# albertfgu/diffwave-sashimi

Measured on AMD Instinct MI355X. Metric: audio samples/sec (generate.py-style reverse-diffusion sampling, T=200), higher is better.
Workload: dtype f32-equivalent (3-term bf16 split, 6 products, fp32 accumulate); 1 GPU; wnet_h256_d36_T200; backbone=wavenet, batch_per_gpu=16, L=16000, T=200, parallelism=independent clips per GPU, no collective, sampler=hipGraph replay, on-device Philox noise

## Files before the change

### diffwave-sashimi_amd/_lib.py

```python
import ctypes
import os

HERE = os.path.dirname(os.path.abspath(__file__))
LIB_PATH = os.environ.get("DWS_LIB") or os.path.join(HERE, "libdws.so")

DWS_OK, DWS_ERR_INVALID, DWS_ERR_UNSUPPORTED, DWS_ERR_HIP, DWS_ERR_STATE = 0, -1, -2, -3, -4
DWS_KIND_WAVENET, DWS_KIND_SASHIMI = 1, 2
DWS_MAX_POOL = 8
DWS_SAMPLER_DDPM, DWS_SAMPLER_DDIM, DWS_SAMPLER_DPMPP2M = 0, 1, 2
DWS_START_AS_GIVEN, DWS_START_QSAMPLE = 0, 1

c_f32p = ctypes.c_void_p


class ModelDesc(ctypes.Structure):
    _fields_ = [
        ("kind", ctypes.c_int32),
        ("in_channels", ctypes.c_int32), ("out_channels", ctypes.c_int32),
        ("diffusion_step_embed_dim_in", ctypes.c_int32),
        ("diffusion_step_embed_dim_mid", ctypes.c_int32),
        ("diffusion_step_embed_dim_out", ctypes.c_int32),
        ("unconditional", ctypes.c_int32),
        ("mel_upsample", ctypes.c_int32 * 2),
        ("mel_bands", ctypes.c_int32),
        ("res_channels", ctypes.c_int32), ("skip_channels", ctypes.c_int32),
        ("num_res_layers", ctypes.c_int32), ("dilation_cycle", ctypes.c_int32),
        ("d_model", ctypes.c_int32), ("n_layers", ctypes.c_int32), ("n_pool", ctypes.c_int32),
        ("pool", ctypes.c_int32 * DWS_MAX_POOL), ("expand", ctypes.c_int32), ("ff", ctypes.c_int32),
        ("unet", ctypes.c_int32), ("L", ctypes.c_int32),
    ]


class SamplerEdit(ctypes.Structure):
    _fields_ = [
        ("edit_coef", ctypes.POINTER(ctypes.c_float)),
        ("known", c_f32p), ("mask", ctypes.c_void_p), ("known_noise", c_f32p), ("start_noise", c_f32p),
        ("start_step", ctypes.c_int32), ("start_mode", ctypes.c_int32),
    ]


_SIGS = {
    "dws_last_error": (ctypes.c_char_p, []),
    "dws_abi_version": (ctypes.c_int, []),
    "dws_arch": (ctypes.c_char_p, []),
    "dws_cauchy_sym_fwd": (ctypes.c_int, [c_f32p] * 4 + [ctypes.c_int64] * 3 + [ctypes.c_void_p]),
    "dws_cauchy_sym_bwd": (ctypes.c_int, [c_f32p] * 6 + [ctypes.c_int64] * 3 + [ctypes.c_void_p]),
    "dws_cauchy_fwd": (ctypes.c_int, [c_f32p] * 4 + [ctypes.c_int64] * 3 + [ctypes.c_void_p]),
    "dws_cauchy_bwd": (ctypes.c_int, [c_f32p] * 6 + [ctypes.c_int64] * 3 + [ctypes.c_void_p]),
    "dws_model_create": (ctypes.c_int, [ctypes.POINTER(ModelDesc), ctypes.POINTER(ctypes.c_void_p)]),
    "dws_model_destroy": (ctypes.c_int, [ctypes.c_void_p]),
    "dws_model_num_params": (ctypes.c_int, [ctypes.c_void_p]),
    "dws_model_param_info": (ctypes.c_int, [ctypes.c_void_p, ctypes.c_int, ctypes.POINTER(ctypes.c_char_p),
                                            ctypes.POINTER(ctypes.c_int64), ctypes.POINTER(ctypes.c_int),
                                            ctypes.POINTER(ctypes.c_int)]),
    "dws_model_set_param": (ctypes.c_int, [ctypes.c_void_p, ctypes.c_char_p, ctypes.c_void_p,
                                           ctypes.POINTER(ctypes.c_int64), ctypes.c_int, ctypes.c_int,
                                           ctypes.c_void_p]),
    "dws_model_update_params": (ctypes.c_int, [ctypes.c_void_p, ctypes.c_int32, ctypes.POINTER(ctypes.c_char_p),
                                               ctypes.POINTER(ctypes.c_void_p), ctypes.c_void_p]),
    "dws_model_set_option": (ctypes.c_int, [ctypes.c_void_p, ctypes.c_char_p, ctypes.c_char_p]),
    "dws_model_commit": (ctypes.c_int, [ctypes.c_void_p, ctypes.c_void_p]),
    "dws_model_prepare": (ctypes.c_int, [ctypes.c_void_p, ctypes.c_int64, ctypes.c_int64]),
    "dws_model_set_condition": (ctypes.c_int, [ctypes.c_void_p, c_f32p, ctypes.c_int64, ctypes.c_int64,
                                               ctypes.c_void_p]),
    "dws_model_forward": (ctypes.c_int, [ctypes.c_void_p, c_f32p, c_f32p, c_f32p, ctypes.c_void_p]),
    "dws_model_forward_train": (ctypes.c_int, [ctypes.c_void_p, c_f32p, c_f32p, c_f32p, ctypes.c_void_p]),
    "dws_model_backward": (ctypes.c_int, [ctypes.c_void_p, c_f32p, ctypes.c_void_p]),
    "dws_model_backward_input": (ctypes.c_int, [ctypes.c_void_p, c_f32p, c_f32p, ctypes.c_int32, ctypes.c_void_p]),
    "dws_model_get_grad": (ctypes.c_int, [ctypes.c_void_p, ctypes.c_char_p, c_f32p, ctypes.c_int64, ctypes.c_void_p]),
    "dws_model_get_grads": (ctypes.c_int, [ctypes.c_void_p, ctypes.c_int32, ctypes.POINTER(ctypes.c_char_p),
                                           ctypes.POINTER(ctypes.c_void_p), ctypes.POINTER(ctypes.c_int64), ctypes.c_void_p]),
    "dws_model_set_grad_sinks": (ctypes.c_int, [ctypes.c_void_p, ctypes.c_int32, ctypes.POINTER(ctypes.c_char_p),
                                                ctypes.POINTER(ctypes.c_void_p), ctypes.POINTER(ctypes.c_int64),
                                                ctypes.POINTER(ctypes.c_int32), ctypes.c_int32]),
    "dws_model_grad_group_wait": (ctypes.c_int, [ctypes.c_void_p, ctypes.c_int32, ctypes.c_void_p]),
    "dws_model_grad_ready_seq": (ctypes.c_int, [ctypes.c_void_p, ctypes.c_int32, ctypes.POINTER(ctypes.c_char_p),
                                                ctypes.POINTER(ctypes.c_int32)]),
    "dws_model_read_tap": (ctypes.c_int, [ctypes.c_void_p, ctypes.c_char_p, c_f32p, ctypes.c_int64, ctypes.c_void_p]),
    "dws_sampler_run": (ctypes.c_int, [ctypes.c_void_p, c_f32p, ctypes.POINTER(ctypes.c_float),
                                       ctypes.POINTER(ctypes.c_float), ctypes.POINTER(ctypes.c_float),
                                       ctypes.c_int32, c_f32p, ctypes.c_uint64, ctypes.c_int32, ctypes.c_int32,
                                       ctypes.c_void_p]),
    "dws_sampler_steps": (ctypes.c_int, [ctypes.c_void_p, c_f32p, ctypes.POINTER(ctypes.c_float),
                                         ctypes.POINTER(ctypes.c_float), ctypes.POINTER(ctypes.c_float),
                                         ctypes.c_int32, ctypes.c_int32, ctypes.c_int32, ctypes.c_uint64,
                                         ctypes.c_int32, ctypes.c_void_p]),
    "dws_sampler_run_schedule": (ctypes.c_int, [ctypes.c_void_p, c_f32p, ctypes.c_int32, ctypes.c_int32,
                                                ctypes.POINTER(ctypes.c_float), ctypes.POINTER(ctypes.c_float), c_f32p,
                                                ctypes.c_uint64, ctypes.c_int32, ctypes.c_int32, ctypes.c_void_p]),
    "dws_sampler_run_edit": (ctypes.c_int, [ctypes.c_void_p, c_f32p, ctypes.c_int32, ctypes.c_int32,
                                            ctypes.POINTER(ctypes.c_float), ctypes.POINTER(ctypes.c_float), c_f32p,
                                            ctypes.c_uint64, ctypes.c_int32, ctypes.c_int32,
                                            ctypes.POINTER(SamplerEdit), ctypes.c_void_p]),
    "dws_sampler_run_program": (ctypes.c_int, [ctypes.c_void_p, c_f32p, ctypes.c_int32, ctypes.c_int32,
                                               ctypes.POINTER(ctypes.c_float), ctypes.POINTER(ctypes.c_float),
                                               ctypes.c_int32, ctypes.POINTER(ctypes.c_int32),
                                               ctypes.POINTER(ctypes.c_float), c_f32p, ctypes.c_uint64, ctypes.c_int32,
                                               ctypes.c_int32, ctypes.POINTER(SamplerEdit), ctypes.c_void_p]),
    "dws_philox_normal": (ctypes.c_int, [c_f32p, ctypes.c_int64, ctypes.c_uint64, ctypes.c_uint32, ctypes.c_void_p]),
    "dws_mel_spectrogram": (ctypes.c_int, [c_f32p, ctypes.c_int64, ctypes.c_int64, c_f32p, c_f32p, ctypes.c_int32,
                                           ctypes.c_int32, ctypes.c_int32, ctypes.c_float, c_f32p, ctypes.c_void_p]),
    "dws_gemm_bf16x6": (ctypes.c_int, [c_f32p] * 3 + [ctypes.c_int64] * 3 + [ctypes.c_void_p]),
    "dws_gemm_f16x3": (ctypes.c_int, [c_f32p] * 3 + [ctypes.c_int64] * 3 + [ctypes.c_float] * 2 + [ctypes.c_void_p]),
    "dws_profile_enable": (ctypes.c_int, [ctypes.c_char_p]),
    "dws_profile_query": (ctypes.c_int, [ctypes.POINTER(ctypes.c_int64), ctypes.POINTER(ctypes.c_double)]),
    "dws_profile_query_each": (ctypes.c_int, [ctypes.POINTER(ctypes.c_double), ctypes.c_int64, ctypes.POINTER(ctypes.c_int64)]),
    "dws_profile_disable": (ctypes.c_int, []),
}

EXPORTS = tuple(_SIGS)

_lib = None


def load():
    global _lib
    if _lib is not None:
        return _lib
    if not os.path.exists(LIB_PATH):
        raise RuntimeError(
            f"{LIB_PATH} not found: the HIP engine is not built (run `python -c 'import __graft_entry__ as g; "
            "g.build()'`).  There is no CPU fallback.")
    lib = ctypes.CDLL(LIB_PATH, mode=ctypes.RTLD_GLOBAL)
    for name, (res, args) in _SIGS.items():
        fn = getattr(lib, name)
        fn.restype, fn.argtypes = res, args
    _lib = lib
    return lib


def check(status):
    if status == DWS_OK:
        return
    msg = load().dws_last_error().decode("utf-8", "replace")
    if status == DWS_ERR_UNSUPPORTED:
        raise NotImplementedError(msg)
    raise RuntimeError(f"libdws error {status}: {msg}")


def ptr(t):
    return 0 if t is None else t.data_ptr()


def current_stream():
    import torch
    return torch.cuda.current_stream().cuda_stream
```

### diffwave-sashimi_amd/csrc/bf16_split.h

```cpp
#pragma once
#include <hip/hip_runtime.h>

namespace dws {

typedef __bf16 bx_bf16x8 __attribute__((ext_vector_type(8)));
typedef __bf16 bx_bf16x4 __attribute__((ext_vector_type(4)));
typedef float bx_f32x16 __attribute__((ext_vector_type(16)));

__device__ __forceinline__ void split3(float x, __bf16& p0, __bf16& p1, __bf16& p2) {
    p0 = (__bf16)x;
    const float r1 = x - (float)p0;
    p1 = (__bf16)r1;
    const float r2 = r1 - (float)p1;
    p2 = (__bf16)r2;
}

__device__ __forceinline__ void split3x4(const float (&x)[4], bx_bf16x4& p0, bx_bf16x4& p1, bx_bf16x4& p2) {
#pragma unroll
    for (int e = 0; e < 4; ++e) {
        __bf16 a, b, c;
        split3(x[e], a, b, c);
        p0[e] = a; p1[e] = b; p2[e] = c;
    }
}

__device__ constexpr int BX6_IA[6] = {2, 1, 0, 1, 0, 0};
__device__ constexpr int BX6_IB[6] = {0, 1, 2, 0, 1, 0};

__device__ __forceinline__ void mfma6(bx_f32x16& acc, const bx_bf16x8 (&a)[3], const bx_bf16x8 (&b)[3]) {
#pragma unroll
    for (int t = 0; t < 6; ++t) acc = __builtin_amdgcn_mfma_f32_32x32x16_bf16(a[BX6_IA[t]], b[BX6_IB[t]], acc, 0, 0, 0);
}

__device__ __forceinline__ void frag_rank2(float v0, float v1, bool lower_half, bx_bf16x8 (&out)[3]) {
    __bf16 a0, a1, a2, b0, b1, b2;
    split3(lower_half ? v0 : 0.f, a0, a1, a2);
    split3(lower_half ? v1 : 0.f, b0, b1, b2);
    const __bf16 z = (__bf16)0.f;
    out[0] = bx_bf16x8{a0, b0, z, z, z, z, z, z};
    out[1] = bx_bf16x8{a1, b1, z, z, z, z, z, z};
    out[2] = bx_bf16x8{a2, b2, z, z, z, z, z, z};
}

struct SplitBf16x3 {
    typedef bx_bf16x8 v8;
    typedef bx_bf16x4 v4;
    static constexpr int NT = 3, NP = 6;
    static constexpr bool SCALED = false;
    static constexpr float SX = 1.f, SG = 1.f;
    __device__ static constexpr int ia(int t) { return BX6_IA[t]; }
    __device__ static constexpr int ib(int t) { return BX6_IB[t]; }
    __device__ static __forceinline__ bx_f32x16 mfma(const v8& a, const v8& b, const bx_f32x16& c) {
        return __builtin_amdgcn_mfma_f32_32x32x16_bf16(a, b, c, 0, 0, 0);
    }
    __device__ static __forceinline__ void split4(const float (&x)[4], v4 (&p)[3]) { split3x4(x, p[0], p[1], p[2]); }
    __device__ static __forceinline__ void split1(float x, v8 (&out)[3], int i) {
        __bf16 a, b, c;
        split3(x, a, b, c);
        out[0][i] = a; out[1][i] = b; out[2][i] = c;
    }
    __device__ static __forceinline__ void rank2(float v0, float v1, bool lower_half, v8 (&out)[3]) { frag_rank2(v0, v1, lower_half, out); }
    __device__ static __forceinline__ void bits(float x, unsigned short (&b)[3]) {
        __bf16 p0, p1, p2;
        split3(x, p0, p1, p2);
        b[0] = __builtin_bit_cast(unsigned short, p0); b[1] = __builtin_bit_cast(unsigned short, p1); b[2] = __builtin_bit_cast(unsigned short, p2);
    }
    __device__ static __forceinline__ v8 bvals(float v0, float v1) {
        const __bf16 z = (__bf16)0.f;
        return v8{(__bf16)v0, (__bf16)v1, z, z, z, z, z, z};
    }
};

typedef _Float16 hx_f16x8 __attribute__((ext_vector_type(8)));
typedef _Float16 hx_f16x4 __attribute__((ext_vector_type(4)));
struct SplitF16x2 {
    typedef hx_f16x8 v8;
    typedef hx_f16x4 v4;
    static constexpr int NT = 2, NP = 3;
    static constexpr bool SCALED = true;
#ifndef F16X3_SX
#define F16X3_SX 16.f
#endif
    static constexpr float SX = F16X3_SX, SG = 4096.f;
    __device__ static constexpr int ia(int t) { return t == 0 ? 1 : 0; }
    __device__ static constexpr int ib(int t) { return t == 1 ? 1 : 0; }
    __device__ static __forceinline__ bx_f32x16 mfma(const v8& a, const v8& b, const bx_f32x16& c) {
        return __builtin_amdgcn_mfma_f32_32x32x16_f16(a, b, c, 0, 0, 0);
    }
    __device__ static __forceinline__ void split4(const float (&x)[4], v4 (&p)[2]) {
#pragma unroll
        for (int e = 0; e < 4; ++e) {
            const _Float16 h = (_Float16)x[e];
            p[0][e] = h;
            p[1][e] = (_Float16)(x[e] - (float)h);
        }
    }
    __device__ static __forceinline__ void split1(float x, v8 (&out)[2], int i) {
        const _Float16 h = (_Float16)x;
        out[0][i] = h;
        out[1][i] = (_Float16)(x - (float)h);
    }
    __device__ static __forceinline__ void bits(float x, unsigned short (&b)[2]) {
        const _Float16 h = (_Float16)x, l = (_Float16)(x - (float)h);
        b[0] = __builtin_bit_cast(unsigned short, h); b[1] = __builtin_bit_cast(unsigned short, l);
    }
    __device__ static __forceinline__ void rank2(float v0, float v1, bool lower_half, v8 (&out)[2]) {
        const _Float16 z = (_Float16)0.f;
        out[0] = v8{z, z, z, z, z, z, z, z};
        out[1] = out[0];
        split1(lower_half ? v0 : 0.f, out, 0);
        split1(lower_half ? v1 : 0.f, out, 1);
    }
    __device__ static __forceinline__ v8 bvals(float v0, float v1) {
        const _Float16 z = (_Float16)0.f;
        return v8{(_Float16)v0, (_Float16)v1, z, z, z, z, z, z};
    }
};

}
```

### diffwave-sashimi_amd/csrc/wavenet.h

```cpp
#pragma once
#include "dws_common.h"

namespace dws {

constexpr int WN_LAYER_KC = 32;
constexpr int WN_BX3_KC = 16;

struct WnLayerArgs {
    const float* x_in;
    float* x_out;
    float* skip;
    const float* part_t;
    int part_t_bstride;
    const float* A1;
    const float* A2;
    const float* Abt;
    int abt_bstride;
    const int* step_idx;
    int abt_tstride, part_t_tstride;
    const float* Wd;
    const float* Wr;
    const float* Ws;
    const float* bias1;
    const float* bias2;
    const float* melc;
    int mel_bstride;
    float* gate_ws;
    float* hsave;
    int B, L, dilation, first_layer, last_layer;
    const float* wscale;
    unsigned long long* trace;
};

struct WnFinalArgs {
    const float* skip;
    const float* Af;
    const float* Wf;
    const float* bf;
    const float* Wz;
    const float* bz;
    float* out;
    float* tap;
    float scale;
    int B, L, Cout;
    int af_scaled;
};

int launch_fold_weight_norm(const float* v, const float* g, float* out, int O, int inner, hipStream_t s);
int launch_permute_dconv(const float* w, float* out, int C, int KC, hipStream_t s);
int launch_pack_a_frag(const float* w, float* out, int M, int K, hipStream_t s);
int launch_pack_a_frag_t(const float* w, float* out, int O, int K, hipStream_t s);
int launch_step_embed(const float* steps, const float* freq, float* emb, int B, int half, hipStream_t s);
int launch_iota_f32(float* out, int n, hipStream_t s);
int launch_linear_rows(const float* in, const float* W, const float* bias, float* out, int B, int K, int O,
                       int act, hipStream_t s, float* pre_out = nullptr);
int launch_init_conv_bwd_data(const float* g, const float* y, const float* W, float* daudio, int B, int Cin, int C, int L,
                              hipStream_t s);
int launch_init_conv(const float* audio, const float* W, const float* bias, float* x, int B, int Cin, int C, int L,
                     hipStream_t s);
int launch_wn_bias_tap(const float* Wd_all, const float* part_t, float* Abt, int NL, int B, int C, hipStream_t s);
bool wn_layer_mfma_supported(int C, int S);
int launch_wn_layer_mfma(int C, int S, const WnLayerArgs& a, hipStream_t s);
int launch_wn_layer_generic(int C, int S, const WnLayerArgs& a, hipStream_t s);
bool wn_final_mfma_supported(int S);
bool wn_layer_wino_supported(int C, int S);
int launch_wino_dconv(const float* w, float* out, int C, hipStream_t s);
int launch_wn_wino_bias(const float* Wd_all, const float* part_t, float* Abt, int NL, int B, int C, hipStream_t s);
int launch_wn_layer_wino(int C, int S, const WnLayerArgs& a, hipStream_t s);
bool wn_layer_bf16x3_supported(int C, int S);
int launch_wn_layer_bf16x3(int C, int S, const WnLayerArgs& a, hipStream_t s);
int launch_pack_a_bf16x3(const float* w, void* out, int M, int K, hipStream_t s);
int launch_wn_bias_tap_bf16(const float* Wd_all, const float* part_t, const float* bias1_all, void* Abt, int NL, int B, int C,
                            hipStream_t s);
enum { WN_SPLIT_BF16X6 = 0, WN_SPLIT_F16X3 = 1 };
inline int wn_split_terms(int split) { return split == WN_SPLIT_F16X3 ? 2 : 3; }
bool wn_layer_bx6_supported(int C, int S);
int launch_wn_layer_bx6(int C, int S, const WnLayerArgs& a, int split, hipStream_t s);
int launch_weight_scale(const float* w, size_t n, const float* bias, int nb, const float* bias_b, int nb_b, float* out, hipStream_t s);
int launch_pack_a1_bx6(const float* w, void* out, int C, int split, const float* scale, hipStream_t s);
int launch_pack_a_bx6(const float* w, void* out, int M, int K, int split, const float* scale, hipStream_t s);
int launch_gemm_bx6(const float* A, const float* B, float* C, int M, int N, int K, int split, float sa, float sb, hipStream_t s);
int launch_wn_final(int S, const WnFinalArgs& a, hipStream_t s);

}
```

### diffwave-sashimi_amd/csrc/wavenet_bx6.hip

```cpp
#include <cstdlib>
#include <type_traits>

#include "bf16_split.h"
#include "wavenet.h"
#include "wn_trace.h"

namespace dws {

#ifndef BX6_PF3
#define BX6_PF3 1
#endif
#ifndef BX6_PF2
#define BX6_PF2 2
#endif
#define BX6_PF(NT) ((NT) == 2 ? BX6_PF2 : BX6_PF3)
#ifndef BX6_T_PER_MFMA
#define BX6_T_PER_MFMA 7
#endif

typedef float bx6_f32x4 __attribute__((ext_vector_type(4)));

#ifdef BX6_ABL_NO_NT
#define BX6_NT 0
#else
#define BX6_NT 2
#endif
__device__ __forceinline__ bx6_f32x4 bx6_load_f4(__amdgpu_buffer_rsrc_t r, int voff, int soff) {
    return __builtin_bit_cast(bx6_f32x4, __builtin_amdgcn_raw_buffer_load_b128(r, voff, soff, BX6_NT));
}
__device__ __forceinline__ void bx6_store_f4(bx6_f32x4 v, __amdgpu_buffer_rsrc_t r, int voff, int soff) {
    typedef unsigned int u4 __attribute__((ext_vector_type(4)));
    __builtin_amdgcn_raw_buffer_store_b128(__builtin_bit_cast(u4, v), r, voff, soff, BX6_NT);
}

__device__ __forceinline__ float bx6_gate(float t, float s) {
    const float tc = __builtin_amdgcn_fmed3f(t, -30.f, 30.f);
    const float e2 = __builtin_amdgcn_exp2f(tc * 2.8853900817779268f);
    const float en = __builtin_amdgcn_exp2f(s * -1.4426950408889634f);
    return (e2 - 1.f) * __builtin_amdgcn_rcpf((e2 + 1.f) * (1.f + en));
}

template <typename P>
__global__ void pack_a1_bx6_kernel(const float* __restrict__ w, unsigned short* __restrict__ out, int C, const float* __restrict__ scale) {
    const size_t i = (size_t)blockIdx.x * blockDim.x + threadIdx.x;
    if (i >= (size_t)2 * C * C * 4) return;
    const int e = (int)(i & 7), lane = (int)((i >> 3) & 63), j = (int)((i >> 9) & 3);
    const size_t r = i >> 11;
    const int nkb = C / 16;
    const int kb = (int)(r % nkb), mt = (int)(r / nkb);
    const int o = mt * 32 + (lane & 31), c = kb * 16 + 8 * (lane >> 5) + e;
    const float* wr = w + ((size_t)o * C + c) * 3;
    const float w0 = wr[0], w1 = wr[1], w2 = wr[2];
    float g;
    if (j == 0) g = w0;
    else if (j == 1) g = 0.5f * ((w0 + w2) + w1);
    else if (j == 2) g = 0.5f * ((w0 + w2) - w1);
    else g = w2;
    if (P::SCALED) g *= *scale;
    unsigned short b[P::NT];
    P::bits(g, b);
    const size_t base = ((r * 4 + j) * P::NT) * 512 + (size_t)lane * 8 + e;
#pragma unroll
    for (int t = 0; t < P::NT; ++t) out[base + t * 512] = b[t];
}

template <typename P>
__global__ void pack_a_bx6_kernel(const float* __restrict__ w, unsigned short* __restrict__ out, int M, int K, const float* __restrict__ scale) {
    const size_t i = (size_t)blockIdx.x * blockDim.x + threadIdx.x;
    if (i >= (size_t)M * K) return;
    const int e = (int)(i & 7), lane = (int)((i >> 3) & 63);
    const size_t r = i >> 9;
    const int nkb = K / 16;
    const int kb = (int)(r % nkb), mt = (int)(r / nkb);
    float v = w[(size_t)(mt * 32 + (lane & 31)) * K + kb * 16 + 8 * (lane >> 5) + e];
    if (P::SCALED) v *= *scale;
    unsigned short b[P::NT];
    P::bits(v, b);
    const size_t base = (r * P::NT) * 512 + (size_t)lane * 8 + e;
#pragma unroll
    for (int t = 0; t < P::NT; ++t) out[base + t * 512] = b[t];
}

__global__ __launch_bounds__(1024) void weight_scale_kernel(const float* __restrict__ w, size_t n, const float* __restrict__ bias, int nb,
                                                            const float* __restrict__ bias_b, int nb_b, float* __restrict__ out) {
    __shared__ float red[16];
    float m = 0.f;
    for (size_t i = threadIdx.x; i < n; i += 1024) m = fmaxf(m, fabsf(w[i]));
    if (bias)
        for (int i = threadIdx.x; i < nb; i += 1024) m = fmaxf(m, fabsf(bias[i]) * (1.f / 1024.f));
    if (bias_b)
        for (int i = threadIdx.x; i < nb_b; i += 1024) m = fmaxf(m, fabsf(bias_b[i]) * (1.f / 1024.f));
#pragma unroll
    for (int o = 32; o > 0; o >>= 1) m = fmaxf(m, __shfl_xor(m, o));
    if ((threadIdx.x & 63) == 0) red[threadIdx.x >> 6] = m;
    __syncthreads();
    if (threadIdx.x == 0) {
        for (int i = 1; i < 16; ++i) m = fmaxf(m, red[i]);
        int ex = 0;
        if (m > 0.f && m < 3.0e38f) {
            frexpf(m, &ex);
            if (ex > 100) ex = 100;
            if (ex < -100) ex = -100;
        }
        *out = ldexpf(1.f, 1 - ex);
    }
}

int launch_weight_scale(const float* w, size_t n, const float* bias, int nb, const float* bias_b, int nb_b, float* out, hipStream_t s) {
    hipLaunchKernelGGL(weight_scale_kernel, dim3(1), dim3(1024), 0, s, w, n, bias, nb, bias_b, nb_b, out);
    return DWS_OK;
}

int launch_pack_a1_bx6(const float* w, void* out, int C, int split, const float* scale, hipStream_t s) {
    const size_t n = (size_t)2 * C * C * 4;
    if (split == WN_SPLIT_F16X3) {
        DWS_CHECK(scale != nullptr, DWS_ERR_INVALID, "pack_a1: the fp16 split needs the matrix scale");
        hipLaunchKernelGGL(pack_a1_bx6_kernel<SplitF16x2>, dim3(ceil_div(n, 256)), dim3(256), 0, s, w, (unsigned short*)out, C, scale);
    } else {
        hipLaunchKernelGGL(pack_a1_bx6_kernel<SplitBf16x3>, dim3(ceil_div(n, 256)), dim3(256), 0, s, w, (unsigned short*)out, C, scale);
    }
    return DWS_OK;
}

int launch_pack_a_bx6(const float* w, void* out, int M, int K, int split, const float* scale, hipStream_t s) {
    DWS_CHECK(M % 32 == 0 && K % 16 == 0, DWS_ERR_UNSUPPORTED, "pack_a_bx6: M=%d K=%d", M, K);
    const size_t n = (size_t)M * K;
    if (split == WN_SPLIT_F16X3) {
        DWS_CHECK(scale != nullptr, DWS_ERR_INVALID, "pack_a: the fp16 split needs the matrix scale");
        hipLaunchKernelGGL(pack_a_bx6_kernel<SplitF16x2>, dim3(ceil_div(n, 256)), dim3(256), 0, s, w, (unsigned short*)out, M, K, scale);
    } else {
        hipLaunchKernelGGL(pack_a_bx6_kernel<SplitBf16x3>, dim3(ceil_div(n, 256)), dim3(256), 0, s, w, (unsigned short*)out, M, K, scale);
    }
    return DWS_OK;
}

template <int C, int S, int NT>
struct Bx6Tile {
    static constexpr int WAVES = C / 32;
    static constexpr int NTH = WAVES * 64;
    static constexpr int NP = 32;
    static constexpr int KC = (C >= 256) ? 32 : 16;
    static constexpr int NCB = C / KC;
    static constexpr int NKB = C / 16;
    static constexpr int MS = S / C;
    static constexpr int RAW_FLOATS = KC * 4 * NP;
    static constexpr int BOP_BYTES = (KC / 8) * 4 * NT * NP * 16;
    static constexpr int STAGE_FLOATS = 2 * RAW_FLOATS + 2 * BOP_BYTES / 4;
    static constexpr int GATE_BYTES = (C / 8) * NT * 64 * 16;
    static constexpr int MAIN_FLOATS = STAGE_FLOATS > GATE_BYTES / 4 ? STAGE_FLOATS : GATE_BYTES / 4;
    static constexpr int TR_FLOATS = 32 * 64;
    static constexpr int LDS_FLOATS = MAIN_FLOATS + WAVES * TR_FLOATS;
    static constexpr int TITEMS = (KC / 4) * NP * 2;
    static_assert(C % 32 == 0 && S % C == 0 && C % KC == 0 && KC % 16 == 0 && KC % (2 * WAVES) == 0 &&
                  (TITEMS % NTH == 0) && LDS_FLOATS * 4 <= 163840, "channel counts");
};

template <typename P, int C, int S, bool EXTRA>
__global__ __launch_bounds__(C * 2, (C >= 128 ? 2 : 1)) void wn_layer_bx6_kernel(WnLayerArgs a, int log2d) {
    using T = Bx6Tile<C, S, P::NT>;
    using v8 = typename P::v8;
    using v4 = typename P::v4;
    constexpr int NT = P::NT, NPR = P::NP, NA = 2 * P::NT;
    constexpr int KC = T::KC, MS = T::MS, WAVES = T::WAVES, NCB = T::NCB, NTH = T::NTH, NKB = T::NKB;
    __shared__ __attribute__((aligned(16))) float lds[T::LDS_FLOATS];
    float* const Xraw = lds;
    char* const Bop = reinterpret_cast<char*>(lds + 2 * T::RAW_FLOATS);
    char* const gt = reinterpret_cast<char*>(lds);

    const int tid = threadIdx.x;
    const int lane = tid & 63;
    const int wave = __builtin_amdgcn_readfirstlane(tid >> 6);
    const int l31 = lane & 31, lhi = lane >> 5;
    const int L = a.L, dil = 1 << log2d;
    float* const trw = lds + T::MAIN_FLOATS + wave * T::TR_FLOATS;

    const int nblk = (L + 2 * dil - 1) >> (log2d + 1);
    const int ntl = ((nblk << log2d) + 31) >> 5;
    const int tile = xcd_remap(blockIdx.x, gridDim.x);
    const int b = __builtin_amdgcn_readfirstlane(tile / ntl);
    const int tic = tile % ntl;
#ifdef WN_TILE_ORDER_LINEAR
    const int q0 = __builtin_amdgcn_readfirstlane(tic * 32);
#else
    const int q0 = __builtin_amdgcn_readfirstlane(log2d >= 6 ? ((tic % nblk) << log2d) + (tic / nblk) * 32 : tic * 32);
#endif
    const int q = q0 + l31;
    const int p = ((q >> log2d) << (log2d + 1)) + (q & (dil - 1));

    const float* __restrict__ xb = a.x_in + (size_t)b * C * L;
    unsigned long long* __restrict__ trc = a.trace ? a.trace + ((size_t)blockIdx.x * WAVES + wave) * 32 : nullptr;
    auto stamp = [&](int i) {
        if (trc) {
            const unsigned long long t = __builtin_amdgcn_s_memtime();
            if (lane == 0) trc[i] = t;
        }
    };
    stamp(0);

    const int mt1[2] = {wave, C / 32 + wave};
    int mt2[1 + MS];
    mt2[0] = wave;
#pragma unroll
    for (int m = 0; m < MS; ++m) mt2[1 + m] = C / 32 + wave * MS + m;
    float av1[2][4], ab1[2], av2[1 + MS];
    {
        const float* Abt = a.Abt + (size_t)b * a.abt_bstride + step_row_off(a.step_idx, a.abt_tstride);
#pragma unroll
        for (int m = 0; m < 2; ++m) {
            const int row = mt1[m] * 32 + l31;
#pragma unroll
            for (int j = 0; j < 4; ++j) av1[m][j] = Abt[j * 2 * C + row];
            ab1[m] = a.bias1[row];
        }
#pragma unroll
        for (int m = 0; m < 1 + MS; ++m) av2[m] = a.bias2[mt2[m] * 32 + l31];
    }
    const float ws1 = P::SCALED ? a.wscale[0] : 1.f, ws2 = P::SCALED ? a.wscale[1] : 1.f;
    const float inv1 = 1.f / (ws1 * P::SX), inv2 = 1.f / (ws2 * P::SG);

    const bool al16 = (L % 4 == 0) && ((((size_t)a.x_in | (size_t)a.x_out | (size_t)a.skip) & 15) == 0);
    const bool contig = al16 && log2d <= 4;
    const bool x4 = contig || (al16 && log2d >= 2);
    constexpr int RPW = KC / WAVES;
    __amdgpu_buffer_rsrc_t rXall = __builtin_amdgcn_make_buffer_rsrc((void*)xb, 0, C * L * 4, 0x00020000);
    const int pbase = (q0 >> log2d) << (log2d + 1);
    const int ob = contig ? 32 + (p - pbase) - dil : l31;
    const int os = contig ? dil : 32;
    const int x0l = p - pbase, x1l = x0l + dil;
    const int gcol0 = contig ? x0l : l31, gcol1 = contig ? x1l : 32 + l31;
    int voffA, voffB;
    if (contig) {
        const int pp = pbase - 32 + 4 * (lane & 31);
        voffA = ((unsigned)pp < (unsigned)L) ? (lhi * L + pp) * 4 : 0x7ffffff0;
        voffB = 0;
    } else if (x4) {
        const int s4 = (lane >> 3) & 3, qq = q0 + 4 * (lane & 7);
        const int pp = ((qq >> log2d) << (log2d + 1)) + (qq & (dil - 1)) + (s4 - 1) * dil;
        voffA = ((unsigned)pp < (unsigned)L) ? (lhi * L + pp) * 4 : 0x7ffffff0;
        voffB = 0;
    } else {
        voffA = (p + (lhi - 1) * dil) * 4;
        voffB = (p + (lhi + 1) * dil) * 4;
    }
#ifdef BX6_ABL_NO_ROT
    const int rot = 0;
#else
    const int rot = __builtin_amdgcn_readfirstlane((int)((unsigned)tic % NCB));
#endif
    auto chunk_of = [&](int cb) { const int c = cb + rot; return c >= NCB ? c - NCB : c; };
    constexpr int NPIECE = RPW / 2;
    auto stage_piece = [&](int cbi, int i) {
        float* xs = Xraw + (cbi & 1) * T::RAW_FLOATS;
        const int cb = chunk_of(cbi);
        {
            const int cc = 2 * (wave + WAVES * i);
            if (x4) {
                __builtin_amdgcn_raw_ptr_buffer_load_lds(rXall, xs + cc * 128, 16, voffA, (cb * KC + cc) * L * 4, 0, BX6_NT);
            } else {
#pragma unroll
                for (int h = 0; h < 2; ++h) {
                    __amdgpu_buffer_rsrc_t r = __builtin_amdgcn_make_buffer_rsrc((void*)(xb + (size_t)(cb * KC + cc + h) * L), 0, L * 4, 0x00020000);
                    __builtin_amdgcn_raw_ptr_buffer_load_lds(r, xs + (cc + h) * 128, 4, voffA, 0, 0, 0);
                    __builtin_amdgcn_raw_ptr_buffer_load_lds(r, xs + (cc + h) * 128 + 64, 4, voffB, 0, 0, 0);
                }
            }
        }
    };
    auto stage_dma = [&](int cbi) {
#pragma unroll
        for (int i = 0; i < NPIECE; ++i) stage_piece(cbi, i);
    };

    auto transform = [&](int c1) {
        const float* xs = Xraw + (c1 & 1) * T::RAW_FLOATS;
        char* bo = Bop + (c1 & 1) * T::BOP_BYTES;
#pragma unroll
        for (int k = 0; k < T::TITEMS / NTH; ++k) {
            const int i = tid + NTH * k;
            const int gi = __builtin_amdgcn_readfirstlane(i >> 6);
            const int g4 = (gi * 2 + lhi) % (KC / 4);
            const int jp = __builtin_amdgcn_readfirstlane((gi * 2) / (KC / 4));
            float ta[4], tb[4];
#pragma unroll
            for (int e = 0; e < 4; ++e) {
                const float* xr = xs + (g4 * 4 + e) * 128 + ob;
                const float d1 = xr[os], d2 = xr[2 * os];
                if (jp == 0) {
                    const float d0 = xr[0];
                    ta[e] = d0 - d2; tb[e] = d1 + d2;
                } else {
                    const float d3 = xr[3 * os];
                    ta[e] = d2 - d1; tb[e] = d1 - d3;
                }
            }
            if (P::SCALED) {
#pragma unroll
                for (int e = 0; e < 4; ++e) { ta[e] *= P::SX; tb[e] *= P::SX; }
            }
            v4 pa[NT], pb[NT];
            P::split4(ta, pa);
            P::split4(tb, pb);
            char* dst = bo + ((((g4 >> 1) * 4 + 2 * jp) * NT) * 32 + l31) * 16 + (g4 & 1) * 8;
#pragma unroll
            for (int t = 0; t < NT; ++t) {
                *reinterpret_cast<v4*>(dst + t * 512) = pa[t];
                *reinterpret_cast<v4*>(dst + (NT + t) * 512) = pb[t];
            }
        }
        if (al16) {
            const int ch0 = chunk_of(c1) * KC;
            if (ch0 / 32 == wave) {
                const int r0 = ch0 % 32;
#pragma unroll
                for (int i = 0; i < KC / 4; ++i) {
                    const int rr = (lane >> 4) + 4 * i;
                    const bx6_f32x4 v = *reinterpret_cast<const bx6_f32x4*>(xs + rr * 128 + 32 + 4 * (lane & 15));
                    *reinterpret_cast<bx6_f32x4*>(trw + (r0 + rr) * 64 + 4 * (lane & 15)) = v;
                }
            }
        }
    };

    bx_f32x16 acc[2][4];
    __amdgpu_buffer_rsrc_t rA1 = __builtin_amdgcn_make_buffer_rsrc((void*)a.A1, 0, 2 * C * 4 * C * 2 * NT, 0x00020000);
    const int lane16 = lane * 16;
    auto load_a1 = [&](v8 (&dst)[2][NT], int kb, int j) {
#pragma unroll
        for (int m = 0; m < 2; ++m)
#pragma unroll
            for (int t = 0; t < NT; ++t)
#ifdef BX6_ABL_A_HOT
                dst[m][t] = __builtin_bit_cast(v8, __builtin_amdgcn_raw_buffer_load_b128(rA1, lane16, ((mt1[m] * NKB * 4) * NT + t) * 1024 + 0 * (kb + j), 0));
#else
                dst[m][t] = __builtin_bit_cast(v8, __builtin_amdgcn_raw_buffer_load_b128(rA1, lane16, (((mt1[m] * NKB + kb) * 4 + j) * NT + t) * 1024, 0));
#endif
    };

    stage_dma(0);
    if (NCB > 1) stage_dma(1);
    constexpr int PF = BX6_PF(NT);
    v8 a_ring[4][2][NT];
#pragma unroll
    for (int s0 = 0; s0 < PF; ++s0) load_a1(a_ring[s0], chunk_of(0) * (KC / 16) + (s0 >> 2), s0 & 3);
    constexpr int NAF = PF * NA;
    if (NCB > 1) {
        if (x4) __builtin_amdgcn_s_waitcnt(0x0F70 | ((RPW / 2 + NAF) & 15) | (((RPW / 2 + NAF) >> 4) << 14));
        else __builtin_amdgcn_s_waitcnt(0x0F70 | ((2 * RPW + NAF) & 15) | (((2 * RPW + NAF) >> 4) << 14));
    } else {
        __builtin_amdgcn_s_waitcnt(0x0F70 | NAF);
    }
    __syncthreads();
    stamp(1);
    {
        const float v0 = ((unsigned)(p - dil) < (unsigned)L) ? 1.f : 0.f;
        const float v1 = ((unsigned)p < (unsigned)L) ? 1.f : 0.f;
        const float v2 = ((unsigned)(p + dil) < (unsigned)L) ? 1.f : 0.f;
        const float v3 = ((unsigned)(p + 2 * dil) < (unsigned)L) ? 1.f : 0.f;
        const float bi[4] = {v0 - v2, v1 + v2, v2 - v1, v1 - v3};
        bx_f32x16 zero;
#pragma unroll
        for (int r = 0; r < 16; ++r) zero[r] = 0.f;
#pragma unroll
        for (int j = 0; j < 4; ++j) {
            const v8 bf = P::bvals(lhi ? 0.f : bi[j] * P::SX, (lhi || j != 1) ? 0.f : P::SX);
#pragma unroll
            for (int m = 0; m < 2; ++m) {
                v8 af[NT];
                P::rank2(av1[m][j] * ws1, j == 1 ? ab1[m] * ws1 : 0.f, lhi == 0, af);
                acc[m][j] = zero;
#pragma unroll
                for (int t = NT - 1; t >= 0; --t) acc[m][j] = P::mfma(af[t], bf, acc[m][j]);
            }
        }
    }
    transform(0);
    __builtin_amdgcn_s_waitcnt(0x0F70 | NAF);
    __syncthreads();

    constexpr int SPC = (KC / 16) * 4;
    auto do_step = [&](int cb, auto ST, auto WITH_T) {
        constexpr int st = decltype(ST)::value;
        constexpr bool with_t = decltype(WITH_T)::value;
        constexpr int it = st >> 2, j = st & 3;
        constexpr int sn = (st + PF) % SPC, itn = sn >> 2, jn = sn & 3;
        const int cbn = cb + (st + PF) / SPC;
        const char* tb = Bop + (cb & 1) * T::BOP_BYTES + lhi * (4 * NT * 512) + l31 * 16;
#if !defined(BX6_ABL_NO_STAGE) && defined(BX6_STAGE_SPREAD)
        if (cb + 2 < NCB) {
            constexpr int NS = (SPC - PF) < 1 ? 1 : (SPC - PF);
#pragma unroll
            for (int i = 0; i < NPIECE; ++i)
                if (i * NS / NPIECE == st) stage_piece(cb + 2, i);
        }
#endif
        if (cbn < NCB) load_a1(a_ring[(st + PF) & 3], chunk_of(cbn) * (KC / 16) + itn, jn);
        __builtin_amdgcn_sched_barrier(0);
        v8 bq[NT];
#pragma unroll
        for (int t = 0; t < NT; ++t) bq[t] = *reinterpret_cast<const v8*>(tb + ((2 * it * 4 + j) * NT + t) * 512);
#ifndef BX6_ABL_NO_TRANSFORM
        if (with_t) transform(cb + 1);
#endif
#pragma unroll
        for (int t = 0; t < NPR; ++t)
#pragma unroll
            for (int m = 0; m < 2; ++m)
                acc[m][j] = P::mfma(a_ring[st & 3][m][P::ia(t)], bq[P::ib(t)], acc[m][j]);
#ifndef BX6_ABL_NO_INTERLEAVE
        if (with_t) {
#pragma unroll
            for (int i = 0; i < 2 * NPR; ++i) {
                __builtin_amdgcn_sched_group_barrier(0x008, 1, 0);
                __builtin_amdgcn_sched_group_barrier(0x302, BX6_T_PER_MFMA * 6 / NPR, 0);
            }
        }
#endif
    };
    auto do_steps_from1 = [&](int cb) {
        if constexpr (SPC == 4) {
            do_step(cb, std::integral_constant<int, 1>{}, std::false_type{});
            do_step(cb, std::integral_constant<int, 2>{}, std::false_type{});
            do_step(cb, std::integral_constant<int, 3>{}, std::false_type{});
        } else {
            do_step(cb, std::integral_constant<int, 1>{}, std::false_type{});
            do_step(cb, std::integral_constant<int, 2>{}, std::false_type{});
            do_step(cb, std::integral_constant<int, 3>{}, std::false_type{});
            do_step(cb, std::integral_constant<int, 4>{}, std::false_type{});
            do_step(cb, std::integral_constant<int, 5>{}, std::false_type{});
            do_step(cb, std::integral_constant<int, 6>{}, std::false_type{});
            do_step(cb, std::integral_constant<int, 7>{}, std::false_type{});
        }
    };
    static_assert((SPC == 4 || SPC == 8) && PF >= 1 && PF <= 3, "steps per chunk, prefetch distance");
    for (int cb = 0; cb < NCB; ++cb) {
#if !defined(BX6_ABL_NO_STAGE) && !defined(BX6_STAGE_SPREAD)
        if (cb + 2 < NCB) stage_dma(cb + 2);
#endif
        if (cb + 1 < NCB) do_step(cb, std::integral_constant<int, 0>{}, std::true_type{});
        else do_step(cb, std::integral_constant<int, 0>{}, std::false_type{});
        do_steps_from1(cb);
        stamp(8 + 2 * cb);
#ifndef BX6_ABL_NO_DMA_WAIT
        __builtin_amdgcn_s_waitcnt(0x0F70 | NAF);
#endif
#ifndef BX6_ABL_NO_BARRIER
        __syncthreads();
#endif
        stamp(9 + 2 * cb);
    }
    stamp(2);

    const int L4 = L * 4;
    const bool first = a.first_layer, last = a.last_layer;
    __amdgpu_buffer_rsrc_t rXo = __builtin_amdgcn_make_buffer_rsrc((void*)(a.x_out + (size_t)b * C * L), 0, C * L * 4, 0x00020000);
    __amdgpu_buffer_rsrc_t rSk = __builtin_amdgcn_make_buffer_rsrc((void*)(a.skip + (size_t)b * S * L), 0, S * L * 4, 0x00020000);
    const int p0 = ((q0 >> log2d) << (log2d + 1)) + (q0 & (dil - 1));
    int voff4;
    {
        const int n4 = (lane & 15) >> 3;
        const int pos4 = (contig ? pbase + 32 * n4 : p0 + n4 * dil) + 4 * (lane & 7);
        voff4 = (pos4 < L) ? ((lane >> 4) * L + pos4) * 4 : 0x7ffffff0;
    }
    constexpr bool PRELOAD = MS == 1;
    const int voff4s = first ? 0x7ffffff0 : voff4;
    auto load_pre = [&](int m, bx6_f32x4 (&dst)[8]) {
#pragma unroll
        for (int i = 0; i < 8; ++i) {
            if (m == 0) dst[i] = *reinterpret_cast<const bx6_f32x4*>(trw + ((lane >> 4) + 4 * i) * 64 + 4 * (lane & 15));
            else dst[i] = bx6_load_f4(rSk, voff4s, ((wave * MS + (m - 1)) * 32 + 4 * i) * L4);
        }
    };
    bx6_f32x4 pre[PRELOAD ? 1 + MS : 1][8];
    if (PRELOAD && al16) {
#pragma unroll
        for (int m = 1; m < 1 + MS; ++m) load_pre(m, pre[PRELOAD ? m : 0]);
    }

    const float* melb = (EXTRA && a.melc) ? a.melc + (size_t)(a.mel_bstride ? b : 0) * 2 * C * L : nullptr;
#pragma unroll
    for (int qd = 0; qd < 4; ++qd) {
        float g0[4], g1[4];
#pragma unroll
        for (int e = 0; e < 4; ++e) {
            const int r = qd * 4 + e;
            const int ch = wave * 32 + e + 8 * qd + 4 * lhi;
#pragma unroll
            for (int n = 0; n < 2; ++n) {
                const int pos = p + n * dil;
                float ht, hs;
                if (n == 0) {
                    ht = (acc[0][0][r] + acc[0][1][r]) + acc[0][2][r];
                    hs = (acc[1][0][r] + acc[1][1][r]) + acc[1][2][r];
                } else {
                    ht = (acc[0][1][r] - acc[0][2][r]) - acc[0][3][r];
                    hs = (acc[1][1][r] - acc[1][2][r]) - acc[1][3][r];
                }
                if (P::SCALED) { ht *= inv1; hs *= inv1; }
                if (EXTRA && melb && pos < L) {
                    ht += melb[(size_t)ch * L + pos];
                    hs += melb[(size_t)(C + ch) * L + pos];
                }
                if (EXTRA && a.hsave && pos < L) {
                    float* __restrict__ hb = a.hsave + (size_t)b * 2 * C * L;
                    hb[(size_t)ch * L + pos] = ht;
                    hb[(size_t)(C + ch) * L + pos] = hs;
                }
                const float g = bx6_gate(ht, hs) * P::SG;
                if (n == 0) g0[e] = g; else g1[e] = g;
            }
        }
        v4 s0[NT], s1[NT];
        P::split4(g0, s0);
        P::split4(g1, s1);
        char* dst = gt + ((wave * 4 + qd) * NT * 64) * 16 + lhi * 8;
#pragma unroll
        for (int t = 0; t < NT; ++t) {
            *reinterpret_cast<v4*>(dst + (t * 64 + gcol0) * 16) = s0[t];
            *reinterpret_cast<v4*>(dst + (t * 64 + gcol1) * 16) = s1[t];
        }
    }
    stamp(3);

    __amdgpu_buffer_rsrc_t rA2 = __builtin_amdgcn_make_buffer_rsrc((void*)a.A2, 0, (C + S) * C * 2 * NT, 0x00020000);
    v8 c_cur[1 + MS][NT], c_nxt[1 + MS][NT];
    auto load_a2 = [&](v8 (&dst)[1 + MS][NT], int kb) {
#pragma unroll
        for (int m = 0; m < 1 + MS; ++m)
#pragma unroll
            for (int t = 0; t < NT; ++t)
                dst[m][t] = __builtin_bit_cast(v8, __builtin_amdgcn_raw_buffer_load_b128(rA2, lane16, ((mt2[m] * NKB + kb) * NT + t) * 1024, 0));
    };
    const int rot2 = rot * (KC / 16);
    auto kblock_of = [&](int kb) { const int k = kb + rot2; return k >= NKB ? k - NKB : k; };
    load_a2(c_cur, kblock_of(0));
    bx_f32x16 acc2[1 + MS][2];
    {
        const v8 bf = P::bvals(lhi ? 0.f : P::SG, 0.f);
        bx_f32x16 zero;
#pragma unroll
        for (int r = 0; r < 16; ++r) zero[r] = 0.f;
#pragma unroll
        for (int m = 0; m < 1 + MS; ++m) {
            v8 af[NT];
            P::rank2(av2[m] * ws2, 0.f, lhi == 0, af);
#pragma unroll
            for (int n = 0; n < 2; ++n) {
                acc2[m][n] = zero;
#pragma unroll
                for (int t = NT - 1; t >= 0; --t) acc2[m][n] = P::mfma(af[t], bf, acc2[m][n]);
            }
        }
    }
    __syncthreads();
    stamp(4);
    const char* gb = gt + lhi * (NT * 64 * 16) + l31 * 16;
#pragma unroll 2
    for (int kb = 0; kb < NKB; ++kb) {
        const int kbn = (kb + 1 < NKB) ? kb + 1 : kb;
        load_a2(c_nxt, kblock_of(kbn));
        __builtin_amdgcn_sched_barrier(0);
        const char* gk = gb + kblock_of(kb) * (2 * NT * 64 * 16);
        v8 bq[2][NT];
#pragma unroll
        for (int n = 0; n < 2; ++n)
#pragma unroll
            for (int t = 0; t < NT; ++t) bq[n][t] = *reinterpret_cast<const v8*>(gk + (t * 64 + n * 32) * 16);
#pragma unroll
        for (int t = 0; t < NPR; ++t)
#pragma unroll
            for (int m = 0; m < 1 + MS; ++m)
#pragma unroll
                for (int n = 0; n < 2; ++n)
                    acc2[m][n] = P::mfma(c_cur[m][P::ia(t)], bq[n][P::ib(t)], acc2[m][n]);
#pragma unroll
        for (int m = 0; m < 1 + MS; ++m)
#pragma unroll
            for (int t = 0; t < NT; ++t) c_cur[m][t] = c_nxt[m][t];
    }
    stamp(5);

    const float rs = 0.70710678118654752440f;
    if (al16) {
#pragma unroll
        for (int m = 0; m < 1 + MS; ++m) {
            if (m == 0 && last) continue;
            if (!PRELOAD || m == 0) load_pre(m, pre[0]);
            asm volatile("s_waitcnt lgkmcnt(0)" ::: "memory");
#pragma unroll
            for (int n = 0; n < 2; ++n)
#pragma unroll
                for (int r = 0; r < 16; ++r) trw[((r & 3) + 8 * (r >> 2) + 4 * lhi) * 64 + n * 32 + l31] = P::SCALED ? acc2[m][n][r] * inv2 : acc2[m][n][r];
            asm volatile("s_waitcnt lgkmcnt(0)" ::: "memory");
            const int row0 = (m == 0) ? wave * 32 : (wave * MS + (m - 1)) * 32;
#pragma unroll
            for (int i = 0; i < 8; ++i) {
                const bx6_f32x4 v = *reinterpret_cast<const bx6_f32x4*>(trw + ((lane >> 4) + 4 * i) * 64 + 4 * (lane & 15));
                bx6_f32x4 o = pre[PRELOAD ? m : 0][i] + v;
                if (m == 0) o = o * rs;
                bx6_store_f4(o, m == 0 ? rXo : rSk, voff4, (row0 + 4 * i) * L4);
                asm volatile("s_nop 1" ::: "memory");
            }
            asm volatile("" ::: "memory");
        }
    } else {
        int voffn[2];
#pragma unroll
        for (int n = 0; n < 2; ++n) {
            const int pos = contig ? pbase + 32 * n + l31 : p + n * dil;
            voffn[n] = (pos < L) ? (4 * lhi * L + pos) * 4 : 0x7ffffff0;
        }
#pragma unroll
        for (int n = 0; n < 2; ++n) {
            if (!last) {
                const int s0 = (wave * 32) * L4;
#pragma unroll
                for (int r = 0; r < 16; ++r) {
                    const int so = s0 + ((r & 3) + 8 * (r >> 2)) * L4;
                    const float x = __builtin_bit_cast(float, __builtin_amdgcn_raw_buffer_load_b32(rXall, voffn[n], so, 0));
                    const float v = (x + (P::SCALED ? acc2[0][n][r] * inv2 : acc2[0][n][r])) * rs;
                    __builtin_amdgcn_raw_buffer_store_b32(__builtin_bit_cast(unsigned, v), rXo, voffn[n], so, 0);
                }
            }
#pragma unroll
            for (int m = 0; m < MS; ++m) {
                const int s0 = ((wave * MS + m) * 32) * L4;
#pragma unroll
                for (int r = 0; r < 16; ++r) {
                    const int so = s0 + ((r & 3) + 8 * (r >> 2)) * L4;
                    const float old = first ? 0.f : __builtin_bit_cast(float, __builtin_amdgcn_raw_buffer_load_b32(rSk, voffn[n], so, 0));
                    const float v = old + (P::SCALED ? acc2[1 + m][n][r] * inv2 : acc2[1 + m][n][r]);
                    __builtin_amdgcn_raw_buffer_store_b32(__builtin_bit_cast(unsigned, v), rSk, voffn[n], so, 0);
                }
            }
        }
    }
    stamp(6);
    if (trc) {
        __builtin_amdgcn_s_waitcnt(0);
        stamp(7);
    }
}

template <typename P, int C, int S>
static int launch_bx6_t(const WnLayerArgs& a, int log2d, hipStream_t s) {
    ProfileScope ps(P::NT == 3 ? "wn_layer_bx6" : "wn_layer_f16x3", s);
    using T = Bx6Tile<C, S, P::NT>;
    const int dil = 1 << log2d;
    const int nblk = (a.L + 2 * dil - 1) / (2 * dil);
    const int ntl = (nblk * dil + 31) / 32;
    const int ntiles = a.B * ntl;
    static const bool trace = std::getenv("DWS_BX6_TRACE") != nullptr;
    if (trace && !a.melc && !a.hsave) {
        wino_trace_launch(ntiles, T::WAVES, a, s, [&](const WnLayerArgs& at) {
            hipLaunchKernelGGL((wn_layer_bx6_kernel<P, C, S, false>), dim3(ntiles), dim3(T::NTH), 0, s, at, log2d);
        }, P::NT == 3 ? "bx6" : "f16x3");
        return DWS_OK;
    }
    if (a.melc || a.hsave) hipLaunchKernelGGL((wn_layer_bx6_kernel<P, C, S, true>), dim3(ntiles), dim3(T::NTH), 0, s, a, log2d);
    else hipLaunchKernelGGL((wn_layer_bx6_kernel<P, C, S, false>), dim3(ntiles), dim3(T::NTH), 0, s, a, log2d);
    return DWS_OK;
}

bool wn_layer_bx6_supported(int C, int S) {
    return (C == 64 && S == 64) || (C == 128 && S == 128) || (C == 128 && S == 256) || (C == 256 && S == 256);
}

template <typename P>
static int launch_bx6_p(int C, int S, const WnLayerArgs& a, int log2d, hipStream_t s) {
    if (C == 64 && S == 64) return launch_bx6_t<P, 64, 64>(a, log2d, s);
    if (C == 128 && S == 128) return launch_bx6_t<P, 128, 128>(a, log2d, s);
    if (C == 128 && S == 256) return launch_bx6_t<P, 128, 256>(a, log2d, s);
    if (C == 256 && S == 256) return launch_bx6_t<P, 256, 256>(a, log2d, s);
    return set_error(DWS_ERR_UNSUPPORTED, "wn_layer_bx6: (C=%d,S=%d) not instantiated", C, S);
}

int launch_wn_layer_bx6(int C, int S, const WnLayerArgs& a, int split, hipStream_t s) {
    int log2d = 0;
    while ((1 << log2d) < a.dilation) ++log2d;
    DWS_CHECK((1 << log2d) == a.dilation, DWS_ERR_UNSUPPORTED, "wn_layer_bx6: dilation %d is not a power of two", a.dilation);
    DWS_CHECK((int64_t)a.L + 4 * (int64_t)a.dilation < ((int64_t)1 << 28), DWS_ERR_UNSUPPORTED, "wn_layer_bx6: L too large");
    DWS_CHECK((int64_t)(C > S ? C : S) * a.L * 4 < ((int64_t)1 << 31), DWS_ERR_UNSUPPORTED,
              "wn_layer_bx6: %d channels x L=%d exceed a 2 GiB tensor per clip", C > S ? C : S, a.L);
    if (split == WN_SPLIT_F16X3) {
        DWS_CHECK(a.hsave == nullptr, DWS_ERR_UNSUPPORTED, "wn_layer_f16x3: the training forward runs with precision=f32 or bf16x6");
        DWS_CHECK(a.wscale != nullptr, DWS_ERR_INVALID, "wn_layer_f16x3: no weight scales");
        return launch_bx6_p<SplitF16x2>(C, S, a, log2d, s);
    }
    return launch_bx6_p<SplitBf16x3>(C, S, a, log2d, s);
}

template <typename P>
__global__ __launch_bounds__(64) void gemm_bx6_kernel(const float* __restrict__ A, const float* __restrict__ B, float* __restrict__ Cm,
                                                      int M, int N, int K, float sa, float sb) {
    using v8 = typename P::v8;
    const int lane = threadIdx.x, l31 = lane & 31, lhi = lane >> 5;
    const int mt = blockIdx.y, nt = blockIdx.x;
    bx_f32x16 acc;
#pragma unroll
    for (int r = 0; r < 16; ++r) acc[r] = 0.f;
    for (int kb = 0; kb < K / 16; ++kb) {
        v8 af[P::NT], bf[P::NT];
#pragma unroll
        for (int e = 0; e < 8; ++e) {
            const int k = kb * 16 + 8 * lhi + e;
            P::split1(A[(size_t)(mt * 32 + l31) * K + k] * sa, af, e);
            P::split1(B[(size_t)k * N + nt * 32 + l31] * sb, bf, e);
        }
#pragma unroll
        for (int t = 0; t < P::NP; ++t) acc = P::mfma(af[P::ia(t)], bf[P::ib(t)], acc);
    }
    const float inv = 1.f / (sa * sb);
#pragma unroll
    for (int r = 0; r < 16; ++r)
        Cm[(size_t)(mt * 32 + (r & 3) + 8 * (r >> 2) + 4 * lhi) * N + nt * 32 + l31] = acc[r] * inv;
}

int launch_gemm_bx6(const float* A, const float* B, float* Cm, int M, int N, int K, int split, float sa, float sb, hipStream_t s) {
    DWS_CHECK(M > 0 && N > 0 && K > 0 && M % 32 == 0 && N % 32 == 0 && K % 16 == 0, DWS_ERR_UNSUPPORTED,
              "gemm_bf16x6 / gemm_f16x3: M=%d N=%d must be multiples of 32, K=%d of 16", M, N, K);
    if (split == WN_SPLIT_F16X3) {
        int ea = 0, eb = 0;
        DWS_CHECK(sa > 0.f && sb > 0.f && frexpf(sa, &ea) == 0.5f && frexpf(sb, &eb) == 0.5f, DWS_ERR_INVALID,
                  "gemm_f16x3: the operand scales must be powers of two (%g, %g)", (double)sa, (double)sb);
        hipLaunchKernelGGL(gemm_bx6_kernel<SplitF16x2>, dim3(N / 32, M / 32), dim3(64), 0, s, A, B, Cm, M, N, K, sa, sb);
    } else {
        hipLaunchKernelGGL(gemm_bx6_kernel<SplitBf16x3>, dim3(N / 32, M / 32), dim3(64), 0, s, A, B, Cm, M, N, K, 1.f, 1.f);
    }
    return DWS_OK;
}

}

extern "C" int dws_gemm_bf16x6(const float* A, const float* B, float* C, int64_t M, int64_t N, int64_t K, void* stream) {
    DWS_CHECK(A && B && C, DWS_ERR_INVALID, "dws_gemm_bf16x6: null argument");
    DWS_CHECK(M <= (1 << 20) && N <= (1 << 20) && K <= (1 << 20), DWS_ERR_UNSUPPORTED, "dws_gemm_bf16x6: dimension too large");
    return dws::launch_gemm_bx6(A, B, C, (int)M, (int)N, (int)K, dws::WN_SPLIT_BF16X6, 1.f, 1.f, (hipStream_t)stream);
}

extern "C" int dws_gemm_f16x3(const float* A, const float* B, float* C, int64_t M, int64_t N, int64_t K, float scale_a, float scale_b,
                              void* stream) {
    DWS_CHECK(A && B && C, DWS_ERR_INVALID, "dws_gemm_f16x3: null argument");
    DWS_CHECK(M <= (1 << 20) && N <= (1 << 20) && K <= (1 << 20), DWS_ERR_UNSUPPORTED, "dws_gemm_f16x3: dimension too large");
    return dws::launch_gemm_bx6(A, B, C, (int)M, (int)N, (int)K, dws::WN_SPLIT_F16X3, scale_a, scale_b, (hipStream_t)stream);
}
```

### diffwave-sashimi_amd/csrc/wavenet_model.hip

```cpp
#include <cmath>

#include "conditioner.h"
#include "model.h"
#include "wavenet.h"
#include "wavenet_backward.h"

namespace dws {

struct WaveNetModel : dws_model {
    int Cin, Cout, C, S, NL, cycle, Ein, Emid, Eout, MB;
    bool cond, mfma_layer, mfma_final;
    bool bf16x3 = false;
    bool bf16x6 = false;
    bool f16x3 = false;
    DevBuf wscale;
    bool wino_opt = true;
    bool wino_fits(int64_t nL) const {
        return (int64_t)std::max(C, S) * nL * 4 < ((int64_t)1 << 31) && nL + 4 * ((int64_t)1 << (cycle - 1)) < ((int64_t)1 << 28);
    }
    bool wino() const { return wino_opt && mfma_layer && !bf16x3 && !bf16x6 && !f16x3 && wn_layer_wino_supported(C, S) && (L == 0 || wino_fits(L)); }
    bool wino_rows() const { return wino() || bf16x6 || f16x3; }

    DevBuf Wi;
    std::vector<DevBuf> A1, Wrs, A2, bias2;
    DevBuf Wd_all;
    DevBuf Abt;
    DevBuf Wt_all, bt_all;
    DevBuf b1_all;
    DevBuf Wf, Af;
    DevBuf freq;
    CopyBatch stack_params, unstack_fc_t;
    bool freq_ready = false;
    DevBuf tmp_pack;
    std::vector<DevBuf> melW0, melW1, melWc;
    DevBuf melc;
    DevBuf mel_u0, mel_u1;
    int64_t melBm = 0;
    DevBuf mel_in;
    int mel_T = 0;
    CondTrainWs cws;
    DevBuf gW0f, gW1f, gWcf;
    DevBuf x0, x1, skip, gate, emb, h1, h2, part_t, scratch_out;
    std::vector<DevBuf> tx, tH;
    std::vector<DevBuf> ATd, ATg;
    std::vector<DevBuf> ATw;
    DevBuf ATf, wpart, bpart;
    bool mfma_bwd = false;
    uint64_t commit_version = 0, bwd_pack_version = ~0ull;
    DevBuf ty, ta1, ta2, dxa, dxb, dskip, dgb, dHb, dresb, dyb, dWfold, dpt, dh2, dh1, demb, dWt_all, dbt_all;
    bool trained_fwd = false;

    explicit WaveNetModel(const dws_model_desc& dd) {
        d = dd;
        Cin = d.in_channels; Cout = d.out_channels; C = d.res_channels; S = d.skip_channels;
        NL = d.num_res_layers; cycle = d.dilation_cycle;
        Ein = d.diffusion_step_embed_dim_in; Emid = d.diffusion_step_embed_dim_mid; Eout = d.diffusion_step_embed_dim_out;
        MB = d.mel_bands;
        cond = !d.unconditional;
        mfma_layer = wn_layer_mfma_supported(C, S);
        mfma_bwd = tapconv_mfma_supported(C, S, C, 1) && tapconv_mfma_supported(C, 2 * C, 0, 3) &&
                   tapconv_mfma_supported(S, S, 0, 1) && std::getenv("DWS_WAVENET_GENERIC_BWD") == nullptr;
        mfma_final = wn_final_mfma_supported(S);
        if (std::getenv("DWS_WN_DIRECT")) wino_opt = false;
        auto wn = [&](const std::string& p, std::vector<int64_t> vshape) {
            std::vector<int64_t> g(vshape.size(), 1);
            g[0] = vshape[0];
            add_param(p + ".bias", {vshape[0]});
            add_param(p + ".weight_g", g);
            add_param(p + ".weight_v", vshape);
        };
        wn("init_conv.0.conv", {C, Cin, 1});
        add_param("residual_layer.fc_t1.weight", {Emid, Ein});
        add_param("residual_layer.fc_t1.bias", {Emid});
        add_param("residual_layer.fc_t2.weight", {Eout, Emid});
        add_param("residual_layer.fc_t2.bias", {Eout});
        for (int n = 0; n < NL; ++n) {
            const std::string p = "residual_layer.residual_blocks." + std::to_string(n);
            add_param(p + ".fc_t.weight", {C, Eout});
            add_param(p + ".fc_t.bias", {C});
            wn(p + ".dilated_conv_layer.conv", {2 * C, C, 3});
            if (cond) {
                for (int i = 0; i < 2; ++i) {
                    const std::string u = p + ".upsample_conv2d." + std::to_string(i);
                    const int s = d.mel_upsample[i];
                    add_param(u + ".bias", {1});
                    add_param(u + ".weight_g", {1, 1, 1, 1});
                    add_param(u + ".weight_v", {1, 1, 3, 2 * s});
                }
                wn(p + ".mel_conv.conv", {2 * C, MB, 1});
            }
            wn(p + ".res_conv", {C, C, 1});
            wn(p + ".skip_conv", {S, C, 1});
        }
        wn("final_conv.0.conv", {S, S, 1});
        add_param("final_conv.2.conv.weight", {Cout, S, 1});
        add_param("final_conv.2.conv.bias", {Cout});
        A1.resize(NL); Wrs.resize(NL); A2.resize(NL); bias2.resize(NL);
        if (cond) { melW0.resize(NL); melW1.resize(NL); melWc.resize(NL); }
    }

    int set_option(const std::string& key, const std::string& value) override {
        if (key == "precision") {
            if (value == "f32") { bf16x3 = bf16x6 = f16x3 = false; dirty = true; trained_fwd = false; return DWS_OK; }
            if (value == "bf16x3") {
                DWS_CHECK(wn_layer_bf16x3_supported(C, S), DWS_ERR_UNSUPPORTED,
                          "precision=bf16x3 is not built for (res_channels=%d, skip_channels=%d)", C, S);
                bf16x3 = true; bf16x6 = f16x3 = false; dirty = true; trained_fwd = false;
                return DWS_OK;
            }
            if (value == "bf16x6") {
                DWS_CHECK(mfma_layer && wn_layer_bx6_supported(C, S), DWS_ERR_UNSUPPORTED,
                          "precision=bf16x6 is not built for (res_channels=%d, skip_channels=%d)", C, S);
                bf16x6 = true; bf16x3 = f16x3 = false; dirty = true; trained_fwd = false;
                return DWS_OK;
            }
            if (value == "f16x3") {
                DWS_CHECK(mfma_layer && wn_layer_bx6_supported(C, S), DWS_ERR_UNSUPPORTED,
                          "precision=f16x3 is not built for (res_channels=%d, skip_channels=%d)", C, S);
                f16x3 = true; bf16x3 = bf16x6 = false; dirty = true; trained_fwd = false;
                return DWS_OK;
            }
        }
        if (key == "conv_algo") {
            if (value == "winograd") { wino_opt = true; dirty = true; trained_fwd = false; return DWS_OK; }
            if (value == "direct") { wino_opt = false; dirty = true; trained_fwd = false; return DWS_OK; }
        }
        return dws_model::set_option(key, value);
    }

    float* Wd(int n) const { return Wd_all.f() + (size_t)n * 2 * C * C * 3; }

    int fold(const std::string& p, float* out, int O, int inner, hipStream_t s) {
        return launch_fold_weight_norm(P(p + ".weight_v"), P(p + ".weight_g"), out, O, inner, s);
    }

    int commit(hipStream_t s) override {
        DWS_TRY(Wi.ensure((size_t)C * Cin * 4));
        DWS_TRY(fold("init_conv.0.conv", Wi.f(), C, Cin, s));
        DWS_TRY(Wt_all.ensure((size_t)NL * C * Eout * 4));
        DWS_TRY(bt_all.ensure((size_t)NL * C * 4));
        DWS_TRY(b1_all.ensure((size_t)NL * 2 * C * 4));
        DWS_TRY(Wd_all.ensure((size_t)NL * 2 * C * C * 3 * 4));
        if (mfma_layer) DWS_TRY(tmp_pack.ensure((size_t)2 * C * 4 * C * 4));
        stack_params.begin();
        for (int n = 0; n < NL; ++n) {
            const std::string p = "residual_layer.residual_blocks." + std::to_string(n);
            stack_params.add(P(p + ".fc_t.weight"), Wt_all.f() + (size_t)n * C * Eout, (size_t)C * Eout);
            stack_params.add(P(p + ".fc_t.bias"), bt_all.f() + (size_t)n * C, (size_t)C);
            stack_params.add(P(p + ".dilated_conv_layer.conv.bias"), b1_all.f() + (size_t)n * 2 * C, (size_t)2 * C);
            DWS_TRY(fold(p + ".dilated_conv_layer.conv", Wd(n), 2 * C, C * 3, s));
            DWS_TRY(Wrs[n].ensure((size_t)(C + S) * C * 4));
            DWS_TRY(fold(p + ".res_conv", Wrs[n].f(), C, C, s));
            DWS_TRY(fold(p + ".skip_conv", Wrs[n].f() + (size_t)C * C, S, C, s));
            DWS_TRY(bias2[n].ensure((size_t)(C + S) * 4));
            stack_params.add(P(p + ".res_conv.bias"), bias2[n].f(), (size_t)C);
            stack_params.add(P(p + ".skip_conv.bias"), bias2[n].f() + C, (size_t)S);
            if (mfma_layer && (bf16x6 || f16x3)) {
                const int split = f16x3 ? WN_SPLIT_F16X3 : WN_SPLIT_BF16X6;
                const size_t tb = 2 * (size_t)wn_split_terms(split);
                float* sc = nullptr;
                if (f16x3) {
                    DWS_TRY(wscale.ensure((size_t)NL * 2 * 4));
                    sc = wscale.f() + 2 * n;
                    DWS_TRY(launch_weight_scale(Wd(n), (size_t)2 * C * C * 3, P(p + ".dilated_conv_layer.conv.bias"), 2 * C, nullptr, 0, sc, s));
                    DWS_TRY(launch_weight_scale(Wrs[n].f(), (size_t)(C + S) * C, P(p + ".res_conv.bias"), C, P(p + ".skip_conv.bias"), S,
                                                sc + 1, s));
                }
                DWS_TRY(A1[n].ensure((size_t)2 * C * 4 * C * tb));
                DWS_TRY(A2[n].ensure((size_t)(C + S) * C * tb));
                DWS_TRY(launch_pack_a1_bx6(Wd(n), A1[n].p, C, split, sc, s));
                DWS_TRY(launch_pack_a_bx6(Wrs[n].f(), A2[n].p, C + S, C, split, f16x3 ? sc + 1 : nullptr, s));
            } else if (mfma_layer) {
                DWS_TRY(A1[n].ensure((size_t)2 * C * 4 * C * 4));
                if (wino()) DWS_TRY(launch_wino_dconv(Wd(n), tmp_pack.f(), C, s));
                else DWS_TRY(launch_permute_dconv(Wd(n), tmp_pack.f(), C, bf16x3 ? WN_BX3_KC : WN_LAYER_KC, s));
                DWS_TRY(A2[n].ensure((size_t)(C + S) * C * 4));
                if (wino()) {
                    DWS_TRY(launch_pack_a_frag(tmp_pack.f(), A1[n].f(), 2 * C, 4 * C, s));
                    DWS_TRY(launch_pack_a_frag(Wrs[n].f(), A2[n].f(), C + S, C, s));
                } else if (bf16x3) {
                    DWS_TRY(launch_pack_a_bf16x3(tmp_pack.f(), A1[n].p, 2 * C, 3 * C, s));
                    DWS_TRY(launch_pack_a_bf16x3(Wrs[n].f(), A2[n].p, C + S, C, s));
                } else {
                    DWS_TRY(launch_pack_a_frag(tmp_pack.f(), A1[n].f(), 2 * C, 3 * C, s));
                    DWS_TRY(launch_pack_a_frag(Wrs[n].f(), A2[n].f(), C + S, C, s));
                }
            }
            if (cond) {
                for (int i = 0; i < 2; ++i) {
                    const int sc = d.mel_upsample[i];
                    DevBuf& w = (i == 0) ? melW0[n] : melW1[n];
                    DWS_TRY(w.ensure((size_t)3 * 2 * sc * 4));
                    DWS_TRY(fold(p + ".upsample_conv2d." + std::to_string(i), w.f(), 1, 3 * 2 * sc, s));
                }
                DWS_TRY(melWc[n].ensure((size_t)2 * C * MB * 4));
                DWS_TRY(fold(p + ".mel_conv.conv", melWc[n].f(), 2 * C, MB, s));
            }
        }
        DWS_TRY(Wf.ensure((size_t)S * S * 4));
        DWS_TRY(fold("final_conv.0.conv", Wf.f(), S, S, s));
        if (mfma_final) {
            DWS_TRY(Af.ensure((size_t)S * S * 4));
            DWS_TRY(tmp_pack.ensure((size_t)std::max(2 * C * 4 * C, S * S) * 4));
            DWS_TRY(launch_scale(Wf.f(), tmp_pack.f(), (float)std::sqrt(1.0 / NL), (size_t)S * S, s));
            DWS_TRY(launch_pack_a_frag(tmp_pack.f(), Af.f(), S, S, s));
        }
        DWS_TRY(stack_params.run(s));
        if (!freq_ready) {
            const int half = Ein / 2;
            std::vector<float> f(half);
            const float e = (float)(-(std::log(10000.0) / (half - 1)));
            for (int i = 0; i < half; ++i) f[i] = (float)std::exp((double)((float)i * e));
            DWS_TRY(freq.ensure((size_t)half * 4));
            DWS_HIP(hipMemcpyAsync(freq.p, f.data(), (size_t)half * 4, hipMemcpyHostToDevice, s));
            DWS_HIP(hipStreamSynchronize(s));
            freq_ready = true;
        }
        if (Abt.p) DWS_HIP(hipMemsetAsync(Abt.p, 0, Abt.bytes, s));
        dirty = false;
        ++commit_version;
        melBm = 0;
        return DWS_OK;
    }

    int pack_bwd(hipStream_t s) {
        const float r2 = 0.70710678118654752440f;
        ATd.resize(NL); ATg.resize(NL); ATw.resize(NL);
        DWS_TRY(tmp_pack.ensure((size_t)std::max(std::max(8 * C * C, (S + C) * C), S * S) * 4));
        for (int n = 0; n < NL; ++n) {
            if (wino_opt && tapwino_mfma_supported(C, 2 * C, 1 << (n % cycle))) {
                DWS_TRY(ATw[n].ensure((size_t)8 * C * C * 4));
                DWS_TRY(launch_tapwino_pack_transposed(Wd(n), tmp_pack.f(), 2 * C, C, s));
                DWS_TRY(launch_pack_a_frag(tmp_pack.f(), ATw[n].f(), C, 8 * C, s));
            } else {
                ATw[n].release();
                DWS_TRY(ATd[n].ensure((size_t)6 * C * C * 4));
                DWS_TRY(launch_tapconv_pack_transposed(Wd(n), tmp_pack.f(), 2 * C, C, 3, 6 * C, 0, 1.f, s));
                DWS_TRY(launch_pack_a_frag(tmp_pack.f(), ATd[n].f(), C, 6 * C, s));
            }
            DWS_TRY(ATg[n].ensure((size_t)(S + C) * C * 4));
            DWS_TRY(launch_tapconv_pack_transposed(Wrs[n].f() + (size_t)C * C, tmp_pack.f(), S, C, 1, S + C, 0, 1.f, s));
            DWS_TRY(launch_tapconv_pack_transposed(Wrs[n].f(), tmp_pack.f(), C, C, 1, S + C, S, r2, s));
            DWS_TRY(launch_pack_a_frag(tmp_pack.f(), ATg[n].f(), C, S + C, s));
        }
        DWS_TRY(ATf.ensure((size_t)S * S * 4));
        DWS_TRY(launch_tapconv_pack_transposed(Wf.f(), tmp_pack.f(), S, S, 1, S, 0, (float)std::sqrt(1.0 / NL), s));
        DWS_TRY(launch_pack_a_frag(tmp_pack.f(), ATf.f(), S, S, s));
        bwd_pack_version = commit_version;
        return DWS_OK;
    }

    int wgrad(const float* dY, const float* X, const float* addc, int addc_bs, float* dW, int O, int Cc, int T, int dil,
              float scale, hipStream_t s, float* db = nullptr, float bscale = 1.f) {
        if (!mfma_bwd) {
            if (db) DWS_TRY(launch_rowsum(dY, db, (int)B, O, (int)L, bscale, 0, s));
            return launch_wgrad(dY, X, addc, addc_bs, dW, (int)B, O, Cc, (int)L, T, dil, scale, s);
        }
        WgradArgs w{};
        w.dY = dY; w.X = X; w.addc = addc; w.addc_bstride = addc_bs;
        w.B = (int)B; w.O = O; w.C = Cc; w.L = (int)L; w.dil = dil;
        w.split = (bf16x6 && O > 1 && Cc > 1) ? 1 : 0;
        const bool wino_w = T == 3 && wino_opt && wgrad_wino_supported(w);
        w.nsplit = wino_w ? wgrad_wino_nsplit((int)B, O, Cc, (int)L, dil) : wgrad_mfma_nsplit((int)B, O, Cc, (int)L, T);
        DWS_TRY(wpart.ensure((size_t)w.nsplit * O * Cc * (wino_w ? 4 : T) * 4));
        w.partial = wpart.f();
        if (db) {
            DWS_TRY(bpart.ensure((size_t)w.nsplit * O * 4));
            w.bias_part = bpart.f(); w.dbias = db; w.bias_scale = bscale;
        }
        if (wino_w) return launch_wgrad_wino(w, scale, dW, s);
        return launch_wgrad_mfma(w, T, scale, dW, s);
    }

    int prepare(int64_t nB, int64_t nL) override {
        DWS_CHECK(nB > 0 && nL > 0, DWS_ERR_INVALID, "prepare: B=%lld L=%lld", (long long)nB, (long long)nL);
        DWS_CHECK(nB * nL * (int64_t)std::max(2 * C, S) < (int64_t)1 << 40, DWS_ERR_UNSUPPORTED, "workspace too large");
        if (nB != B || nL != L) { drop_graph(); melBm = 0; trained_fwd = false; }
        if ((L == 0 || wino_fits(L)) != wino_fits(nL)) dirty = true;
        B = nB; L = nL;
        const size_t act = (size_t)B * C * L * 4;
        DWS_TRY(x0.ensure(act));
        DWS_TRY(x1.ensure(act));
        DWS_TRY(skip.ensure((size_t)B * S * L * 4));
        if (!mfma_layer) DWS_TRY(gate.ensure(act));
        DWS_TRY(emb.ensure((size_t)B * Ein * 4));
        DWS_TRY(h1.ensure((size_t)B * Emid * 4));
        DWS_TRY(h2.ensure((size_t)B * Eout * 4));
        DWS_TRY(part_t.ensure((size_t)B * NL * C * 4));
        if (mfma_layer) {
            const size_t n = (size_t)NL * B * (2 * C / 32) * 2048;
            DWS_TRY(Abt.ensure(n));
            DWS_HIP(hipMemset(Abt.p, 0, n));
        }
        return DWS_OK;
    }

    int set_condition(const float* mel, int64_t Bm, int64_t Tmel, hipStream_t s) override {
        if (mel == nullptr) { melBm = 0; return DWS_OK; }
        DWS_CHECK(cond, DWS_ERR_INVALID, "set_condition on an unconditional model (`wavenet.py:99`)");
        DWS_CHECK(B > 0, DWS_ERR_STATE, "set_condition before prepare");
        DWS_CHECK(Bm == 1 || Bm == B, DWS_ERR_INVALID, "mel batch %lld must be 1 or B=%lld", (long long)Bm, (long long)B);
        if (dirty) DWS_TRY(commit(s));
        const int s0 = d.mel_upsample[0], s1 = d.mel_upsample[1];
        const int T0 = mel_upsampled_len((int)Tmel, s0), T1 = mel_upsampled_len(T0, s1);
        DWS_CHECK(T1 >= L, DWS_ERR_INVALID, "upsampled mel length %d < L=%lld (`wavenet.py:105`)", T1, (long long)L);
        DWS_TRY(mel_u0.ensure((size_t)Bm * MB * T0 * 4));
        DWS_TRY(mel_u1.ensure((size_t)Bm * MB * T1 * 4));
        DWS_TRY(melc.ensure((size_t)NL * Bm * 2 * C * L * 4));
        for (int n = 0; n < NL; ++n) {
            const std::string p = "residual_layer.residual_blocks." + std::to_string(n);
            DWS_TRY(launch_mel_upsample(mel, melW0[n].f(), P(p + ".upsample_conv2d.0.bias"), mel_u0.f(), (int)Bm, MB,
                                        (int)Tmel, T0, s0, 0.4f, s));
            DWS_TRY(launch_mel_upsample(mel_u0.f(), melW1[n].f(), P(p + ".upsample_conv2d.1.bias"), mel_u1.f(), (int)Bm,
                                        MB, T0, T1, s1, 0.4f, s));
            DWS_TRY(launch_conv1x1_trunc(mel_u1.f(), melWc[n].f(), P(p + ".mel_conv.conv.bias"),
                                         melc.f() + (size_t)n * Bm * 2 * C * L, (int)Bm, MB, 2 * C, T1, (int)L, s));
        }
        DWS_TRY(mel_in.ensure((size_t)Bm * MB * Tmel * 4));
        DWS_HIP(hipMemcpyAsync(mel_in.p, mel, (size_t)Bm * MB * Tmel * 4, hipMemcpyDeviceToDevice, s));
        mel_T = (int)Tmel;
        melBm = Bm;
        return DWS_OK;
    }

    int final_stage(float* out, float* tap, hipStream_t s) {
        WnFinalArgs f{};
        f.skip = skip.f(); f.Af = Af.f(); f.Wf = Wf.f(); f.bf = P("final_conv.0.conv.bias");
        f.Wz = P("final_conv.2.conv.weight"); f.bz = P("final_conv.2.conv.bias");
        f.out = out; f.tap = tap; f.scale = (float)std::sqrt(1.0 / NL); f.af_scaled = mfma_final ? 1 : 0;
        f.B = (int)B; f.L = (int)L; f.Cout = Cout;
        return launch_wn_final(S, f, s);
    }

    int forward(const float* audio, const float* steps, float* out, hipStream_t s) override {
        trained_fwd = false;
        return run_forward(audio, steps, out, false, s);
    }

    int forward_train(const float* audio, const float* steps, float* out, hipStream_t s) override {
        DWS_CHECK(B > 0, DWS_ERR_STATE, "forward before prepare");
        DWS_CHECK(!bf16x3 && !f16x3 && (!bf16x6 || mfma_bwd), DWS_ERR_UNSUPPORTED,
                  "training runs with precision=f32, or bf16x6 where the MFMA adjoints run (no bf16x3 / f16x3 backward is built)");
        DWS_CHECK(melBm == 0 || (melBm == B && mfma_bwd), DWS_ERR_UNSUPPORTED,
                  "mel-conditional training needs one mel per clip (got %lld for B=%lld) and the MFMA adjoints (channels %% 32 == 0)",
                  (long long)melBm, (long long)B);
        DWS_CHECK(!cond || melBm > 0, DWS_ERR_STATE, "conditional model: install the mel (set_condition) before forward_train");
        const size_t act = (size_t)B * C * L * 4;
        tx.resize(NL + 1); tH.resize(NL);
        for (int n = 0; n <= NL; ++n) DWS_TRY(tx[n].ensure(act));
        for (int n = 0; n < NL; ++n) DWS_TRY(tH[n].ensure(2 * act));
        DWS_TRY(ty.ensure((size_t)B * S * L * 4));
        DWS_TRY(ta1.ensure((size_t)B * Emid * 4));
        DWS_TRY(ta2.ensure((size_t)B * Eout * 4));
        DWS_TRY(run_forward(audio, steps, out, true, s));
        train_audio = audio;
        trained_fwd = true;
        return DWS_OK;
    }

    const float* train_audio = nullptr;

    int abt_row() const { return wino_rows() ? 4 * 2 * C : (2 * C / 32) * (bf16x3 ? 512 : 256); }

    int embed_rows(const float* steps, int rows, float* emb_, float* h1_, float* h2_, float* pt, void* abt, float* pre1,
                   float* pre2, hipStream_t s) {
        DWS_TRY(launch_step_embed(steps, freq.f(), emb_, rows, Ein / 2, s));
        DWS_TRY(launch_linear_rows(emb_, P("residual_layer.fc_t1.weight"), P("residual_layer.fc_t1.bias"), h1_, rows, Ein, Emid,
                                   1, s, pre1));
        DWS_TRY(launch_linear_rows(h1_, P("residual_layer.fc_t2.weight"), P("residual_layer.fc_t2.bias"), h2_, rows, Emid, Eout,
                                   1, s, pre2));
        DWS_TRY(launch_linear_rows(h2_, Wt_all.f(), bt_all.f(), pt, rows, Eout, NL * C, 0, s));
        if (mfma_layer && bf16x3) DWS_TRY(launch_wn_bias_tap_bf16(Wd_all.f(), pt, b1_all.f(), abt, NL, rows, C, s));
        else if (wino_rows()) DWS_TRY(launch_wn_wino_bias(Wd_all.f(), pt, (float*)abt, NL, rows, C, s));
        else if (mfma_layer) DWS_TRY(launch_wn_bias_tap(Wd_all.f(), pt, (float*)abt, NL, rows, C, s));
        return DWS_OK;
    }

    DevBuf tab_steps, tab_emb, tab_h1, tab_h2, tab_pt, tab_abt;
    int tab_T = 0;
    uint64_t tab_version = ~0ull;
    StepKey tab_key;
    int build_step_table(int T, const float* steps, hipStream_t s) override {
        if (dirty) DWS_TRY(commit(s));
        if (tab_version == commit_version && tab_key.same(T, steps)) return DWS_OK;
        drop_graph();
        {
            const size_t bytes = (size_t)T * ((size_t)NL * C + (mfma_layer ? (size_t)NL * abt_row() : 0) + Ein + Emid + Eout + 1) * 4;
            DWS_CHECK(T > 0 && bytes <= ((size_t)4 << 30), DWS_ERR_UNSUPPORTED,
                      "sampler step table: T=%d needs %.2f GB (limit 4 GB): sample with fewer steps or per-step forwards", T, bytes / 1e9);
        }
        DWS_TRY(tab_steps.ensure((size_t)T * 4));
        DWS_TRY(tab_emb.ensure((size_t)T * Ein * 4));
        DWS_TRY(tab_h1.ensure((size_t)T * Emid * 4));
        DWS_TRY(tab_h2.ensure((size_t)T * Eout * 4));
        DWS_TRY(tab_pt.ensure((size_t)T * NL * C * 4));
        if (mfma_layer) {
            const size_t n = (size_t)NL * T * abt_row() * 4;
            DWS_TRY(tab_abt.ensure(n));
            DWS_HIP(hipMemsetAsync(tab_abt.p, 0, n, s));
        }
        tab_version = ~0ull;
        DWS_TRY(tab_key.upload(T, steps, tab_steps.f(), s));
        DWS_TRY(embed_rows(tab_steps.f(), T, tab_emb.f(), tab_h1.f(), tab_h2.f(), tab_pt.f(), tab_abt.p, nullptr, nullptr, s));
        tab_T = T;
        tab_version = commit_version;
        ++step_table_gen;
        return DWS_OK;
    }

    int run_forward(const float* audio, const float* steps, float* out, bool train, hipStream_t s) {
        DWS_CHECK(B > 0, DWS_ERR_STATE, "forward before prepare");
        if (dirty) DWS_TRY(commit(s));
        const bool tab = step_idx != nullptr && !train;
        DWS_CHECK(!tab || (tab_T > 0 && tab_version == commit_version), DWS_ERR_STATE, "step-table forward without a current table");
        DWS_CHECK(tab || steps, DWS_ERR_INVALID, "forward: steps == null");
        float* xfirst = train ? tx[0].f() : x0.f();
        DWS_TRY(launch_init_conv(audio, Wi.f(), P("init_conv.0.conv.bias"), xfirst, (int)B, Cin, C, (int)L, s));
        if (!tab)
            DWS_TRY(embed_rows(steps, (int)B, emb.f(), h1.f(), h2.f(), part_t.f(), Abt.p, train ? ta1.f() : nullptr,
                               train ? ta2.f() : nullptr, s));
        const int arow = abt_row();
        for (int n = 0; n < NL; ++n) {
            const std::string p = "residual_layer.residual_blocks." + std::to_string(n);
            WnLayerArgs a{};
            a.x_in = train ? tx[n].f() : ((n & 1) ? x1.f() : x0.f());
            a.x_out = train ? tx[n + 1].f() : ((n & 1) ? x0.f() : x1.f());
            a.hsave = train ? tH[n].f() : nullptr;
            a.skip = skip.f();
            a.A1 = A1[n].f(); a.A2 = A2[n].f();
            if (tab) {
                a.part_t = tab_pt.f() + (size_t)n * C; a.part_t_bstride = 0; a.part_t_tstride = NL * C;
                a.Abt = mfma_layer ? tab_abt.f() + (size_t)n * tab_T * arow : nullptr; a.abt_bstride = 0; a.abt_tstride = arow;
                a.step_idx = step_idx;
            } else {
                a.part_t = part_t.f() + (size_t)n * C; a.part_t_bstride = NL * C;
                a.Abt = mfma_layer ? Abt.f() + (size_t)n * B * arow : nullptr; a.abt_bstride = arow;
            }
            a.Wd = Wd(n); a.Wr = Wrs[n].f(); a.Ws = Wrs[n].f() + (size_t)C * C;
            a.bias1 = P(p + ".dilated_conv_layer.conv.bias");
            a.bias2 = bias2[n].f();
            a.melc = melBm ? melc.f() + (size_t)n * melBm * 2 * C * L : nullptr;
            a.mel_bstride = (melBm > 1) ? 1 : 0;
            a.gate_ws = gate.f();
            a.B = (int)B; a.L = (int)L;
            a.dilation = 1 << (n % cycle);
            a.first_layer = (n == 0); a.last_layer = (n == NL - 1);
            if (mfma_layer && bf16x3) DWS_TRY(launch_wn_layer_bf16x3(C, S, a, s));
            else if (bf16x6) DWS_TRY(launch_wn_layer_bx6(C, S, a, WN_SPLIT_BF16X6, s));
            else if (f16x3) { a.wscale = wscale.f() + 2 * n; DWS_TRY(launch_wn_layer_bx6(C, S, a, WN_SPLIT_F16X3, s)); }
            else if (wino()) DWS_TRY(launch_wn_layer_wino(C, S, a, s));
            else if (mfma_layer) DWS_TRY(launch_wn_layer_mfma(C, S, a, s));
            else DWS_TRY(launch_wn_layer_generic(C, S, a, s));
        }
        DWS_TRY(final_stage(out, train ? ty.f() : nullptr, s));
        DWS_HIP(hipGetLastError());
        return DWS_OK;
    }

    int wn_bwd(const std::string& p, const float* dWf, int O, int inner, hipStream_t s) {
        return launch_weight_norm_bwd(dWf, P(p + ".weight_v"), P(p + ".weight_g"), G(p + ".weight_v"), G(p + ".weight_g"), O,
                                      inner, s);
    }

    int backward(const float* dout, float* daudio, bool pg, hipStream_t s) override {
        DWS_CHECK(trained_fwd, DWS_ERR_STATE, "backward without a preceding forward_train");
        DWS_CHECK(pg || daudio, DWS_ERR_INVALID, "backward: a data-only pass needs a destination for the input gradient");
        const int nB = (int)B, nL = (int)L;
        const size_t act = (size_t)B * C * L * 4, nact = (size_t)B * C * L;
        DWS_TRY(dxa.ensure(act)); DWS_TRY(dxb.ensure(act)); DWS_TRY(dgb.ensure(act)); DWS_TRY(dresb.ensure(act));
        DWS_TRY(gate.ensure(act));
        DWS_TRY(dHb.ensure(2 * act));
        DWS_TRY(dskip.ensure((size_t)B * S * L * 4)); DWS_TRY(dyb.ensure((size_t)B * S * L * 4));
        if (pg) {
            DWS_TRY(dWfold.ensure((size_t)std::max(2 * C * C * 3, std::max((C + S) * C, S * S)) * 4));
            DWS_TRY(dpt.ensure((size_t)B * NL * C * 4));
            DWS_TRY(dh2.ensure((size_t)B * Eout * 4)); DWS_TRY(dh1.ensure((size_t)B * Emid * 4));
            DWS_TRY(dWt_all.ensure((size_t)NL * C * Eout * 4)); DWS_TRY(dbt_all.ensure((size_t)NL * C * 4));
        }
        const float scale = (float)std::sqrt(1.0 / NL);

        if (pg) DWS_TRY(wgrad(dout, ty.f(), nullptr, 0, G("final_conv.2.conv.weight"), Cout, S, 1, 1, 1.f, s, G("final_conv.2.conv.bias")));
        DWS_TRY(launch_final_dy(dout, P("final_conv.2.conv.weight"), ty.f(), dyb.f(), nB, S, Cout, nL, s));
        if (pg) {
            DWS_TRY(wgrad(dyb.f(), skip.f(), nullptr, 0, dWfold.f(), S, S, 1, 1, scale, s, G("final_conv.0.conv.bias")));
            DWS_TRY(wn_bwd("final_conv.0.conv", dWfold.f(), S, S, s));
        }
        if (mfma_bwd) {
            if (bwd_pack_version != commit_version) DWS_TRY(pack_bwd(s));
            TapConvArgs f{};
            f.src0 = dyb.f(); f.K0 = S; f.A = ATf.f(); f.nkg_total = S / 8; f.M = S; f.T = 1; f.dil = 1; f.sign = 1;
            f.out = dskip.f(); f.B = nB; f.L = nL; f.split = bf16x6 ? 1 : 0;
            DWS_TRY(launch_tapconv_mfma(f, s));
        } else {
            DWS_TRY(launch_conv_t(dyb.f(), Wf.f(), dskip.f(), nB, S, S, nL, 1, 1, scale, 0, s));
        }

        float* dx_out = nullptr;
        for (int n = NL - 1; n >= 0; --n) {
            const std::string p = "residual_layer.residual_blocks." + std::to_string(n);
            const int dil = 1 << (n % cycle);
            const float* Wr = Wrs[n].f();
            const float* Ws = Wrs[n].f() + (size_t)C * C;
            const float r2 = 0.70710678118654752440f;
            float* dh = (dx_out == dxa.f()) ? dxb.f() : dxa.f();
            if (mfma_bwd) {
                TapConvArgs q{};
                q.src0 = dskip.f(); q.K0 = S; q.src1 = dx_out; q.K1 = dx_out ? C : 0;
                q.A = ATg[n].f(); q.nkg_total = (S + C) / 8; q.M = C; q.T = 1; q.dil = 1; q.sign = 1; q.epi = 1;
                q.H = tH[n].f(); q.dH = dHb.f(); q.g = gate.f(); q.B = nB; q.L = nL; q.split = bf16x6 ? 1 : 0;
                DWS_TRY(launch_tapconv_mfma(q, s));
            } else {
                if (dx_out) {
                    DWS_TRY(launch_scale(dx_out, dresb.f(), r2, nact, s));
                    DWS_TRY(launch_conv_t(dresb.f(), Wr, dgb.f(), nB, C, C, nL, 1, 1, 1.f, 0, s));
                    DWS_TRY(launch_conv_t(dskip.f(), Ws, dgb.f(), nB, S, C, nL, 1, 1, 1.f, 1, s));
                } else {
                    DWS_TRY(launch_conv_t(dskip.f(), Ws, dgb.f(), nB, S, C, nL, 1, 1, 1.f, 0, s));
                }
                DWS_TRY(launch_gate_bwd(dgb.f(), tH[n].f(), dHb.f(), gate.f(), nB, C, nL, s));
            }
            if (melBm && pg) {
                const int s0 = d.mel_upsample[0], s1 = d.mel_upsample[1];
                DWS_TRY(gW0f.ensure((size_t)3 * 2 * s0 * 4)); DWS_TRY(gW1f.ensure((size_t)3 * 2 * s1 * 4));
                DWS_TRY(gWcf.ensure((size_t)2 * C * MB * 4));
                DWS_TRY(conditioner_backward(cws, mel_in.f(), nB, MB, mel_T, s0, s1, melW0[n].f(), P(p + ".upsample_conv2d.0.bias"),
                                             melW1[n].f(), P(p + ".upsample_conv2d.1.bias"), melWc[n].f(), 2 * C, nL, dHb.f(),
                                             gW0f.f(), G(p + ".upsample_conv2d.0.bias"), gW1f.f(),
                                             G(p + ".upsample_conv2d.1.bias"), gWcf.f(), s));
                DWS_TRY(wn_bwd(p + ".upsample_conv2d.0", gW0f.f(), 1, 3 * 2 * s0, s));
                DWS_TRY(wn_bwd(p + ".upsample_conv2d.1", gW1f.f(), 1, 3 * 2 * s1, s));
                DWS_TRY(wn_bwd(p + ".mel_conv.conv", gWcf.f(), 2 * C, MB, s));
            }
            if (pg && dx_out) {
                DWS_TRY(wgrad(dx_out, gate.f(), nullptr, 0, dWfold.f(), C, C, 1, 1, r2, s, G(p + ".res_conv.bias"), r2));
                DWS_TRY(wn_bwd(p + ".res_conv", dWfold.f(), C, C, s));
            } else if (pg) {
                DWS_HIP(hipMemsetAsync(G(p + ".res_conv.weight_v"), 0, (size_t)C * C * 4, s));
                DWS_HIP(hipMemsetAsync(G(p + ".res_conv.weight_g"), 0, (size_t)C * 4, s));
                DWS_HIP(hipMemsetAsync(G(p + ".res_conv.bias"), 0, (size_t)C * 4, s));
            }
            if (pg) {
                DWS_TRY(wgrad(dskip.f(), gate.f(), nullptr, 0, dWfold.f(), S, C, 1, 1, 1.f, s, G(p + ".skip_conv.bias")));
                DWS_TRY(wn_bwd(p + ".skip_conv", dWfold.f(), S, C, s));
                DWS_TRY(wgrad(dHb.f(), tx[n].f(), part_t.f() + (size_t)n * C, NL * C, dWfold.f(), 2 * C, C, 3, dil, 1.f, s,
                              G(p + ".dilated_conv_layer.conv.bias")));
                DWS_TRY(wn_bwd(p + ".dilated_conv_layer.conv", dWfold.f(), 2 * C, C * 3, s));
                if (melBm)
                    DWS_HIP(hipMemcpyAsync(G(p + ".mel_conv.conv.bias"), G(p + ".dilated_conv_layer.conv.bias"), (size_t)2 * C * 4,
                                           hipMemcpyDeviceToDevice, s));
            }
            if (mfma_bwd) {
                TapConvArgs q{};
                q.src0 = dHb.f(); q.K0 = 2 * C; q.A = ATd[n].f(); q.nkg_total = 6 * C / 8; q.M = C; q.T = 3; q.dil = dil;
                q.sign = -1; q.out = dh; q.B = nB; q.L = nL;
                if (wino_opt && tapwino_mfma_supported(C, 2 * C, dil) && ATw[n].p) {
                    q.A = ATw[n].f(); q.nkg_total = C; q.split = bf16x6 ? 1 : 0;
                    DWS_TRY(launch_tapwino_mfma(q, s));
                } else {
                    DWS_CHECK(ATd[n].p, DWS_ERR_STATE, "backward: layer %d's direct adjoint weights were not packed", n);
                    DWS_TRY(launch_tapconv_mfma(q, s));
                }
            } else {
                DWS_TRY(launch_conv_t(dHb.f(), Wd(n), dh, nB, 2 * C, C, nL, 3, dil, 1.f, 0, s));
            }
            if (pg) DWS_TRY(launch_rowsum_bc(dh, dpt.f() + (size_t)n * C, NL * C, nB, C, nL, s));
            if (dx_out) DWS_TRY(launch_dx_combine(dh, dx_out, nact, s));
            dx_out = dh;
            if (pg) DWS_TRY(grad_point(s));
        }
        if (!pg) {
            DWS_TRY(launch_init_conv_bwd_data(dx_out, tx[0].f(), Wi.f(), daudio, nB, Cin, C, nL, s));
            DWS_HIP(hipGetLastError());
            return DWS_OK;
        }
        DWS_TRY(launch_relu_bwd(dx_out, tx[0].f(), nact, s));
        DWS_TRY(wgrad(dx_out, train_audio, nullptr, 0, dWfold.f(), C, Cin, 1, 1, 1.f, s, G("init_conv.0.conv.bias")));
        DWS_TRY(wn_bwd("init_conv.0.conv", dWfold.f(), C, Cin, s));
        if (daudio) DWS_TRY(launch_init_conv_bwd_data(dx_out, nullptr, Wi.f(), daudio, nB, Cin, C, nL, s));

        DWS_TRY(launch_lin_bwd_w(dpt.f(), h2.f(), dWt_all.f(), dbt_all.f(), nB, Eout, NL * C, s));
        unstack_fc_t.begin();
        for (int n = 0; n < NL; ++n) {
            const std::string p = "residual_layer.residual_blocks." + std::to_string(n);
            unstack_fc_t.add(dWt_all.f() + (size_t)n * C * Eout, G(p + ".fc_t.weight"), (size_t)C * Eout);
            unstack_fc_t.add(dbt_all.f() + (size_t)n * C, G(p + ".fc_t.bias"), (size_t)C);
        }
        DWS_TRY(unstack_fc_t.run(s));
        DWS_TRY(launch_lin_bwd_x(dpt.f(), Wt_all.f(), ta2.f(), dh2.f(), nB, Eout, NL * C, lin_scratch, s));
        DWS_TRY(launch_lin_bwd_w(dh2.f(), h1.f(), G("residual_layer.fc_t2.weight"), G("residual_layer.fc_t2.bias"), nB, Emid,
                                 Eout, s));
        DWS_TRY(launch_lin_bwd_x(dh2.f(), P("residual_layer.fc_t2.weight"), ta1.f(), dh1.f(), nB, Emid, Eout, lin_scratch, s));
        DWS_TRY(launch_lin_bwd_w(dh1.f(), emb.f(), G("residual_layer.fc_t1.weight"), G("residual_layer.fc_t1.bias"), nB, Ein,
                                 Emid, s));
        DWS_HIP(hipGetLastError());
        return DWS_OK;
    }

    int read_tap(const char* tap, float* dst, int64_t capacity, hipStream_t s) override {
        DWS_CHECK(B > 0, DWS_ERR_STATE, "read_tap before prepare/forward");
        const std::string t(tap);
        if (t == "skip") {
            DWS_CHECK(capacity >= B * S * L, DWS_ERR_INVALID, "tap buffer too small");
            DWS_HIP(hipMemcpyAsync(dst, skip.p, (size_t)B * S * L * 4, hipMemcpyDeviceToDevice, s));
            return DWS_OK;
        }
        if (t == "x") {
            DWS_CHECK(capacity >= B * C * L, DWS_ERR_INVALID, "tap buffer too small");
            const float* src = ((NL - 1) & 1) ? x1.f() : x0.f();
            DWS_HIP(hipMemcpyAsync(dst, src, (size_t)B * C * L * 4, hipMemcpyDeviceToDevice, s));
            return DWS_OK;
        }
        if (t == "split_launches") {
            DWS_CHECK(capacity >= 2, DWS_ERR_INVALID, "tap buffer too small");
            const bool sp = mfma_layer && (bf16x3 || bf16x6 || f16x3);
            const float v[2] = {sp ? (float)NL : 0.f, sp ? 0.f : (float)NL};
            DWS_HIP(hipMemcpyAsync(dst, v, 8, hipMemcpyHostToDevice, s));
            DWS_HIP(hipStreamSynchronize(s));
            return DWS_OK;
        }
        if (t == "pre_final") {
            DWS_CHECK(capacity >= B * S * L, DWS_ERR_INVALID, "tap buffer too small");
            DWS_TRY(scratch_out.ensure((size_t)B * Cout * L * 4));
            return final_stage(scratch_out.f(), dst, s);
        }
        struct { const char* name; const DevBuf* buf; size_t n; } small[] = {
            {"emb", &emb, (size_t)B * Ein}, {"emb_mlp", &h2, (size_t)B * Eout},
            {"part_t", &part_t, (size_t)B * NL * C}, {"abt", &Abt, mfma_layer ? (size_t)NL * B * abt_row() : 0},
            {"tab_part_t", &tab_pt, (size_t)tab_T * NL * C}, {"tab_abt", &tab_abt, mfma_layer ? (size_t)NL * tab_T * abt_row() : 0}};
        for (auto& e : small)
            if (t == e.name) {
                DWS_CHECK(e.buf->p && e.n > 0 && capacity >= (int64_t)e.n, DWS_ERR_INVALID, "tap '%s': %zu floats, capacity %lld",
                          tap, e.n, (long long)capacity);
                DWS_HIP(hipMemcpyAsync(dst, e.buf->p, e.n * 4, hipMemcpyDeviceToDevice, s));
                return DWS_OK;
            }
        return set_error(DWS_ERR_INVALID, "unknown tap '%s'", tap);
    }
};

dws_model* make_wavenet(const dws_model_desc& d) { return new WaveNetModel(d); }

}
```

### include/dws.h

```cpp
#ifndef DWS_H_
#define DWS_H_

#include <stdint.h>

#ifdef __cplusplus
extern "C" {
#endif

#define DWS_OK               0
#define DWS_ERR_INVALID     -1
#define DWS_ERR_UNSUPPORTED -2
#define DWS_ERR_HIP         -3
#define DWS_ERR_STATE       -4

const char* dws_last_error(void);
int dws_abi_version(void);
const char* dws_arch(void);


int dws_cauchy_sym_fwd(const float* v, const float* z, const float* w, float* out,
                       int64_t B, int64_t N, int64_t L, void* stream);

int dws_cauchy_sym_bwd(const float* v, const float* z, const float* w, const float* dout,
                       float* dv, float* dw, int64_t B, int64_t N, int64_t L, void* stream);

int dws_cauchy_fwd(const float* v, const float* z, const float* w, float* out,
                   int64_t B, int64_t N, int64_t L, void* stream);

int dws_cauchy_bwd(const float* v, const float* z, const float* w, const float* dout,
                   float* dv, float* dw, int64_t B, int64_t N, int64_t L, void* stream);


#define DWS_KIND_WAVENET 1
#define DWS_KIND_SASHIMI 2
#define DWS_MAX_POOL 8

typedef struct dws_model_desc {
    int32_t kind;
    int32_t in_channels, out_channels;
    int32_t diffusion_step_embed_dim_in, diffusion_step_embed_dim_mid, diffusion_step_embed_dim_out;
    int32_t unconditional;
    int32_t mel_upsample[2];
    int32_t mel_bands;
    int32_t res_channels, skip_channels, num_res_layers, dilation_cycle;
    int32_t d_model, n_layers, n_pool, pool[DWS_MAX_POOL], expand, ff, unet, L;
} dws_model_desc;

typedef struct dws_model dws_model;

int dws_model_create(const dws_model_desc* desc, dws_model** out);
int dws_model_destroy(dws_model* m);

int dws_model_num_params(const dws_model* m);
int dws_model_param_info(const dws_model* m, int index, const char** name,
                         int64_t* shape, int* ndim, int* dtype);

int dws_model_set_param(dws_model* m, const char* name, const void* data,
                        const int64_t* shape, int ndim, int dtype, void* stream);

int dws_model_update_params(dws_model* m, int32_t count, const char* const* names, const float* const* srcs, void* stream);

int dws_model_set_option(dws_model* m, const char* key, const char* value);

int dws_model_commit(dws_model* m, void* stream);

int dws_model_prepare(dws_model* m, int64_t B, int64_t L);

int dws_model_set_condition(dws_model* m, const float* mel, int64_t Bm, int64_t Tmel, void* stream);

int dws_model_forward(dws_model* m, const float* audio, const float* steps, float* out, void* stream);

int dws_model_forward_train(dws_model* m, const float* audio, const float* steps, float* out, void* stream);
int dws_model_backward(dws_model* m, const float* dout, void* stream);
int dws_model_backward_input(dws_model* m, const float* dout, float* daudio, int32_t param_grads, void* stream);
int dws_model_get_grad(dws_model* m, const char* name, float* dst, int64_t numel, void* stream);
int dws_model_get_grads(dws_model* m, int32_t count, const char* const* names, float* const* dsts, const int64_t* numels,
                        void* stream);

int dws_model_set_grad_sinks(dws_model* m, int32_t count, const char* const* names, float* const* dsts, const int64_t* numels,
                             const int32_t* groups, int32_t ngroups);
int dws_model_grad_group_wait(dws_model* m, int32_t group, void* waiting_stream);
int dws_model_grad_ready_seq(dws_model* m, int32_t count, const char* const* names, int32_t* seq_out);

int dws_model_read_tap(dws_model* m, const char* tap, float* dst, int64_t capacity, void* stream);

int dws_sampler_run(dws_model* m, float* x, const float* alpha, const float* alpha_bar,
                    const float* sigma, int32_t T, const float* noise, uint64_t seed,
                    int32_t init_from_seed, int32_t use_graph, void* stream);

int dws_sampler_steps(dws_model* m, float* x, const float* alpha, const float* alpha_bar,
                      const float* sigma, int32_t T, int32_t t_start, int32_t n_steps,
                      uint64_t seed, int32_t use_graph, void* stream);

#define DWS_SAMPLER_DDPM 0
#define DWS_SAMPLER_DDIM 1
#define DWS_SAMPLER_DPMPP2M 2
int dws_sampler_run_schedule(dws_model* m, float* x, int32_t kind, int32_t S, const float* net_steps,
                             const float* coef, const float* noise, uint64_t seed, int32_t init_from_seed,
                             int32_t use_graph, void* stream);

#define DWS_START_AS_GIVEN 0
#define DWS_START_QSAMPLE  1
typedef struct dws_sampler_edit {
    const float*   edit_coef;
    const float*   known;
    const uint8_t* mask;
    const float*   known_noise;
    const float*   start_noise;
    int32_t        start_step;
    int32_t        start_mode;
} dws_sampler_edit;
int dws_sampler_run_edit(dws_model* m, float* x, int32_t kind, int32_t S, const float* net_steps,
                         const float* coef, const float* noise, uint64_t seed, int32_t init_from_seed,
                         int32_t use_graph, const dws_sampler_edit* edit, void* stream);

int dws_sampler_run_program(dws_model* m, float* x, int32_t kind, int32_t S, const float* net_steps,
                            const float* coef, int32_t V, const int32_t* visit_step, const float* jump_coef,
                            const float* noise, uint64_t seed, int32_t init_from_seed, int32_t use_graph,
                            const dws_sampler_edit* edit, void* stream);

int dws_philox_normal(float* x, int64_t n, uint64_t seed, uint32_t stream_id, void* stream);

int dws_mel_spectrogram(const float* audio, int64_t B, int64_t T, const float* window, const float* mel_basis,
                        int32_t n_fft, int32_t hop, int32_t n_mels, float clip, float* out, void* stream);

int dws_gemm_bf16x6(const float* A, const float* B, float* C, int64_t M, int64_t N, int64_t K, void* stream);

int dws_gemm_f16x3(const float* A, const float* B, float* C, int64_t M, int64_t N, int64_t K, float scale_a, float scale_b,
                   void* stream);

int dws_profile_enable(const char* substr);
int dws_profile_query(int64_t* launches, double* total_ms);
int dws_profile_query_each(double* ms, int64_t capacity, int64_t* launches);
int dws_profile_disable(void);

#ifdef __cplusplus
}
#endif
#endif
```

Before: 32710 audio samples/s.

## Add 16x16x32 MFMA variant for bf16x6 WaveNet layer at C=S=256

```diff
diff --git a/diffwave-sashimi_amd/_lib.py b/diffwave-sashimi_amd/_lib.py
--- a/diffwave-sashimi_amd/_lib.py
+++ b/diffwave-sashimi_amd/_lib.py
@@ -101,6 +101,7 @@
     "dws_mel_spectrogram": (ctypes.c_int, [c_f32p, ctypes.c_int64, ctypes.c_int64, c_f32p, c_f32p, ctypes.c_int32,
                                            ctypes.c_int32, ctypes.c_int32, ctypes.c_float, c_f32p, ctypes.c_void_p]),
     "dws_gemm_bf16x6": (ctypes.c_int, [c_f32p] * 3 + [ctypes.c_int64] * 3 + [ctypes.c_void_p]),
+    "dws_gemm_bf16x6_k32": (ctypes.c_int, [c_f32p] * 3 + [ctypes.c_int64] * 3 + [ctypes.c_void_p]),
     "dws_gemm_f16x3": (ctypes.c_int, [c_f32p] * 3 + [ctypes.c_int64] * 3 + [ctypes.c_float] * 2 + [ctypes.c_void_p]),
     "dws_profile_enable": (ctypes.c_int, [ctypes.c_char_p]),
     "dws_profile_query": (ctypes.c_int, [ctypes.POINTER(ctypes.c_int64), ctypes.POINTER(ctypes.c_double)]),
diff --git a/diffwave-sashimi_amd/csrc/bf16_split.h b/diffwave-sashimi_amd/csrc/bf16_split.h
--- a/diffwave-sashimi_amd/csrc/bf16_split.h
+++ b/diffwave-sashimi_amd/csrc/bf16_split.h
@@ -117,4 +117,54 @@
     }
 };
 
+typedef float bx_f32x4 __attribute__((ext_vector_type(4)));
+
+struct Mfma32x32x16 {
+    static constexpr int TM = 32, TN = 32, TK = 16;
+    static constexpr int ACCN = 16;
+    typedef bx_f32x16 acc_t;
+    __device__ static __forceinline__ int rc(int lane) { return lane & 31; }
+    __device__ static __forceinline__ int ko(int lane) { return lane >> 5; }
+    __device__ static __forceinline__ int arow(int lane, int r) { return (r & 3) + 8 * (r >> 2) + 4 * (lane >> 5); }
+    __device__ static __forceinline__ acc_t mfma(const bx_bf16x8& a, const bx_bf16x8& b, const acc_t& c) {
+        return __builtin_amdgcn_mfma_f32_32x32x16_bf16(a, b, c, 0, 0, 0);
+    }
+    __device__ static __forceinline__ acc_t mfma(const hx_f16x8& a, const hx_f16x8& b, const acc_t& c) {
+        return __builtin_amdgcn_mfma_f32_32x32x16_f16(a, b, c, 0, 0, 0);
+    }
+};
+
+struct Mfma16x16x32 {
+    static constexpr int TM = 16, TN = 16, TK = 32;
+    static constexpr int ACCN = 4;
+    typedef bx_f32x4 acc_t;
+    __device__ static __forceinline__ int rc(int lane) { return lane & 15; }
+    __device__ static __forceinline__ int ko(int lane) { return lane >> 4; }
+    __device__ static __forceinline__ int arow(int lane, int r) { return 4 * (lane >> 4) + r; }
+    __device__ static __forceinline__ acc_t mfma(const bx_bf16x8& a, const bx_bf16x8& b, const acc_t& c) {
+        return __builtin_amdgcn_mfma_f32_16x16x32_bf16(a, b, c, 0, 0, 0);
+    }
+    __device__ static __forceinline__ acc_t mfma(const hx_f16x8& a, const hx_f16x8& b, const acc_t& c) {
+        return __builtin_amdgcn_mfma_f32_16x16x32_f16(a, b, c, 0, 0, 0);
+    }
+};
+
+template <typename M>
+struct Acc32 {
+    static constexpr int MI = 32 / M::TM, NI = 32 / M::TN, NSUB = MI * NI;
+    static constexpr int GPS = M::ACCN / 4;
+    static_assert(NSUB * GPS == 4, "a lane holds 16 values of a 32 x 32 block");
+    typename M::acc_t sub[NSUB];
+    __device__ static constexpr int ci(int g) { return (g / GPS) % NI; }
+    __device__ static __forceinline__ int row4(int lane, int g) { return M::TM * ((g / GPS) / NI) + M::arow(lane, (g % GPS) * 4); }
+    __device__ static __forceinline__ int col(int lane, int g) { return M::TN * ci(g) + M::rc(lane); }
+    __device__ __forceinline__ float at(int g, int e) const { return sub[g / GPS][(g % GPS) * 4 + e]; }
+    __device__ __forceinline__ void clear() {
+#pragma unroll
+        for (int i = 0; i < NSUB; ++i)
+#pragma unroll
+            for (int r = 0; r < M::ACCN; ++r) sub[i][r] = 0.f;
+    }
+};
+
 }
diff --git a/diffwave-sashimi_amd/csrc/wavenet.h b/diffwave-sashimi_amd/csrc/wavenet.h
--- a/diffwave-sashimi_amd/csrc/wavenet.h
+++ b/diffwave-sashimi_amd/csrc/wavenet.h
@@ -75,10 +75,15 @@
 enum { WN_SPLIT_BF16X6 = 0, WN_SPLIT_F16X3 = 1 };
 inline int wn_split_terms(int split) { return split == WN_SPLIT_F16X3 ? 2 : 3; }
 bool wn_layer_bx6_supported(int C, int S);
-int launch_wn_layer_bx6(int C, int S, const WnLayerArgs& a, int split, hipStream_t s);
+enum { WN_MFMA_32X32X16 = 0, WN_MFMA_16X16X32 = 1 };
+bool wn_layer_bx6_k32_supported(int C, int S, int split);
+int launch_wn_layer_bx6(int C, int S, const WnLayerArgs& a, int split, hipStream_t s, int mfma = WN_MFMA_32X32X16);
 int launch_weight_scale(const float* w, size_t n, const float* bias, int nb, const float* bias_b, int nb_b, float* out, hipStream_t s);
 int launch_pack_a1_bx6(const float* w, void* out, int C, int split, const float* scale, hipStream_t s);
 int launch_pack_a_bx6(const float* w, void* out, int M, int K, int split, const float* scale, hipStream_t s);
+int launch_pack_a1_bx6_k32(const float* w, void* out, int C, hipStream_t s);
+int launch_pack_a_bx6_k32(const float* w, void* out, int M, int K, hipStream_t s);
+int launch_gemm_bx6_k32(const float* A, const float* B, float* C, int M, int N, int K, hipStream_t s);
 int launch_gemm_bx6(const float* A, const float* B, float* C, int M, int N, int K, int split, float sa, float sb, hipStream_t s);
 int launch_wn_final(int S, const WnFinalArgs& a, hipStream_t s);
 
diff --git a/diffwave-sashimi_amd/csrc/wavenet_bx6.hip b/diffwave-sashimi_amd/csrc/wavenet_bx6.hip
--- a/diffwave-sashimi_amd/csrc/wavenet_bx6.hip
+++ b/diffwave-sashimi_amd/csrc/wavenet_bx6.hip
@@ -16,6 +16,9 @@
 #define BX6_PF(NT) ((NT) == 2 ? BX6_PF2 : BX6_PF3)
 #ifndef BX6_T_PER_MFMA
 #define BX6_T_PER_MFMA 7
+#endif
+#ifndef BX6_T_PER_MFMA_K32
+#define BX6_T_PER_MFMA_K32 4
 #endif
 
 typedef float bx6_f32x4 __attribute__((ext_vector_type(4)));
@@ -40,15 +43,15 @@
     return (e2 - 1.f) * __builtin_amdgcn_rcpf((e2 + 1.f) * (1.f + en));
 }
 
-template <typename P>
+template <typename P, typename M>
 __global__ void pack_a1_bx6_kernel(const float* __restrict__ w, unsigned short* __restrict__ out, int C, const float* __restrict__ scale) {
     const size_t i = (size_t)blockIdx.x * blockDim.x + threadIdx.x;
     if (i >= (size_t)2 * C * C * 4) return;
     const int e = (int)(i & 7), lane = (int)((i >> 3) & 63), j = (int)((i >> 9) & 3);
     const size_t r = i >> 11;
-    const int nkb = C / 16;
+    const int nkb = C / M::TK;
     const int kb = (int)(r % nkb), mt = (int)(r / nkb);
-    const int o = mt * 32 + (lane & 31), c = kb * 16 + 8 * (lane >> 5) + e;
+    const int o = mt * M::TM + M::rc(lane), c = kb * M::TK + 8 * M::ko(lane) + e;
     const float* wr = w + ((size_t)o * C + c) * 3;
     const float w0 = wr[0], w1 = wr[1], w2 = wr[2];
     float g;
@@ -64,15 +67,15 @@
     for (int t = 0; t < P::NT; ++t) out[base + t * 512] = b[t];
 }
 
-template <typename P>
-__global__ void pack_a_bx6_kernel(const float* __restrict__ w, unsigned short* __restrict__ out, int M, int K, const float* __restrict__ scale) {
+template <typename P, typename M>
+__global__ void pack_a_bx6_kernel(const float* __restrict__ w, unsigned short* __restrict__ out, int Mr, int K, const float* __restrict__ scale) {
     const size_t i = (size_t)blockIdx.x * blockDim.x + threadIdx.x;
-    if (i >= (size_t)M * K) return;
+    if (i >= (size_t)Mr * K) return;
     const int e = (int)(i & 7), lane = (int)((i >> 3) & 63);
     const size_t r = i >> 9;
-    const int nkb = K / 16;
+    const int nkb = K / M::TK;
     const int kb = (int)(r % nkb), mt = (int)(r / nkb);
-    float v = w[(size_t)(mt * 32 + (lane & 31)) * K + kb * 16 + 8 * (lane >> 5) + e];
+    float v = w[(size_t)(mt * M::TM + M::rc(lane)) * K + kb * M::TK + 8 * M::ko(lane) + e];
     if (P::SCALED) v *= *scale;
     unsigned short b[P::NT];
     P::bits(v, b);
@@ -115,9 +118,9 @@
     const size_t n = (size_t)2 * C * C * 4;
     if (split == WN_SPLIT_F16X3) {
         DWS_CHECK(scale != nullptr, DWS_ERR_INVALID, "pack_a1: the fp16 split needs the matrix scale");
-        hipLaunchKernelGGL(pack_a1_bx6_kernel<SplitF16x2>, dim3(ceil_div(n, 256)), dim3(256), 0, s, w, (unsigned short*)out, C, scale);
+        hipLaunchKernelGGL((pack_a1_bx6_kernel<SplitF16x2, Mfma32x32x16>), dim3(ceil_div(n, 256)), dim3(256), 0, s, w, (unsigned short*)out, C, scale);
     } else {
-        hipLaunchKernelGGL(pack_a1_bx6_kernel<SplitBf16x3>, dim3(ceil_div(n, 256)), dim3(256), 0, s, w, (unsigned short*)out, C, scale);
+        hipLaunchKernelGGL((pack_a1_bx6_kernel<SplitBf16x3, Mfma32x32x16>), dim3(ceil_div(n, 256)), dim3(256), 0, s, w, (unsigned short*)out, C, scale);
     }
     return DWS_OK;
 }
@@ -127,10 +130,26 @@
     const size_t n = (size_t)M * K;
     if (split == WN_SPLIT_F16X3) {
         DWS_CHECK(scale != nullptr, DWS_ERR_INVALID, "pack_a: the fp16 split needs the matrix scale");
-        hipLaunchKernelGGL(pack_a_bx6_kernel<SplitF16x2>, dim3(ceil_div(n, 256)), dim3(256), 0, s, w, (unsigned short*)out, M, K, scale);
+        hipLaunchKernelGGL((pack_a_bx6_kernel<SplitF16x2, Mfma32x32x16>), dim3(ceil_div(n, 256)), dim3(256), 0, s, w, (unsigned short*)out, M, K, scale);
     } else {
-        hipLaunchKernelGGL(pack_a_bx6_kernel<SplitBf16x3>, dim3(ceil_div(n, 256)), dim3(256), 0, s, w, (unsigned short*)out, M, K, scale);
-    }
+        hipLaunchKernelGGL((pack_a_bx6_kernel<SplitBf16x3, Mfma32x32x16>), dim3(ceil_div(n, 256)), dim3(256), 0, s, w, (unsigned short*)out, M, K, scale);
+    }
+    return DWS_OK;
+}
+
+int launch_pack_a1_bx6_k32(const float* w, void* out, int C, hipStream_t s) {
+    DWS_CHECK(C % 32 == 0, DWS_ERR_UNSUPPORTED, "pack_a1_bx6_k32: C=%d", C);
+    const size_t n = (size_t)2 * C * C * 4;
+    hipLaunchKernelGGL((pack_a1_bx6_kernel<SplitBf16x3, Mfma16x16x32>), dim3(ceil_div(n, 256)), dim3(256), 0, s, w, (unsigned short*)out, C,
+                       (const float*)nullptr);
+    return DWS_OK;
+}
+
+int launch_pack_a_bx6_k32(const float* w, void* out, int M, int K, hipStream_t s) {
+    DWS_CHECK(M % 16 == 0 && K % 32 == 0, DWS_ERR_UNSUPPORTED, "pack_a_bx6_k32: M=%d K=%d", M, K);
+    const size_t n = (size_t)M * K;
+    hipLaunchKernelGGL((pack_a_bx6_kernel<SplitBf16x3, Mfma16x16x32>), dim3(ceil_div(n, 256)), dim3(256), 0, s, w, (unsigned short*)out, M, K,
+                       (const float*)nullptr);
     return DWS_OK;
 }
 
@@ -155,13 +174,21 @@
                   (TITEMS % NTH == 0) && LDS_FLOATS * 4 <= 163840, "channel counts");
 };
 
-template <typename P, int C, int S, bool EXTRA>
+template <typename P, typename M, int C, int S, bool EXTRA>
 __global__ __launch_bounds__(C * 2, (C >= 128 ? 2 : 1)) void wn_layer_bx6_kernel(WnLayerArgs a, int log2d) {
     using T = Bx6Tile<C, S, P::NT>;
     using v8 = typename P::v8;
     using v4 = typename P::v4;
+    using Acc = Acc32<M>;
     constexpr int NT = P::NT, NPR = P::NP, NA = 2 * P::NT;
-    constexpr int KC = T::KC, MS = T::MS, WAVES = T::WAVES, NCB = T::NCB, NTH = T::NTH, NKB = T::NKB;
+    constexpr int KC = T::KC, MS = T::MS, WAVES = T::WAVES, NCB = T::NCB, NTH = T::NTH;
+    constexpr int MI = Acc::MI, NI = Acc::NI;
+    constexpr bool SPLIT_M = MI > 1;
+    static_assert(MI == 1 || MI == 2, "a unit carries two A fragments per term");
+    constexpr int NKB = C / M::TK;
+    constexpr int KBC = KC / M::TK;
+    constexpr int KO = M::TK / 8;
+    static_assert(KC % M::TK == 0 && (!SPLIT_M || MS == 1), "chunk / k-block, skip tiles per wave");
     __shared__ __attribute__((aligned(16))) float lds[T::LDS_FLOATS];
     float* const Xraw = lds;
     char* const Bop = reinterpret_cast<char*>(lds + 2 * T::RAW_FLOATS);
@@ -171,6 +198,7 @@
     const int lane = tid & 63;
     const int wave = __builtin_amdgcn_readfirstlane(tid >> 6);
     const int l31 = lane & 31, lhi = lane >> 5;
+    const int frc = M::rc(lane), fko = M::ko(lane);
     const int L = a.L, dil = 1 << log2d;
     float* const trw = lds + T::MAIN_FLOATS + wave * T::TR_FLOATS;
 
@@ -202,18 +230,18 @@
     mt2[0] = wave;
 #pragma unroll
     for (int m = 0; m < MS; ++m) mt2[1 + m] = C / 32 + wave * MS + m;
-    float av1[2][4], ab1[2], av2[1 + MS];
+    float av1[2][MI][4], ab1[2][MI];
     {
         const float* Abt = a.Abt + (size_t)b * a.abt_bstride + step_row_off(a.step_idx, a.abt_tstride);
 #pragma unroll
-        for (int m = 0; m < 2; ++m) {
-            const int row = mt1[m] * 32 + l31;
-#pragma unroll
-            for (int j = 0; j < 4; ++j) av1[m][j] = Abt[j * 2 * C + row];
-            ab1[m] = a.bias1[row];
-        }
-#pragma unroll
-        for (int m = 0; m < 1 + MS; ++m) av2[m] = a.bias2[mt2[m] * 32 + l31];
+        for (int m = 0; m < 2; ++m)
+#pragma unroll
+            for (int mi = 0; mi < MI; ++mi) {
+                const int row = mt1[m] * 32 + mi * M::TM + frc;
+#pragma unroll
+                for (int j = 0; j < 4; ++j) av1[m][mi][j] = Abt[j * 2 * C + row];
+                ab1[m][mi] = a.bias1[row];
+            }
     }
     const float ws1 = P::SCALED ? a.wscale[0] : 1.f, ws2 = P::SCALED ? a.wscale[1] : 1.f;
     const float inv1 = 1.f / (ws1 * P::SX), inv2 = 1.f / (ws2 * P::SG);
@@ -226,8 +254,10 @@
     const int pbase = (q0 >> log2d) << (log2d + 1);
     const int ob = contig ? 32 + (p - pbase) - dil : l31;
     const int os = contig ? dil : 32;
-    const int x0l = p - pbase, x1l = x0l + dil;
-    const int gcol0 = contig ? x0l : l31, gcol1 = contig ? x1l : 32 + l31;
+    auto col_pos = [&](int ni) {
+        const int qc = q0 + M::TN * ni + frc;
+        return ((qc >> log2d) << (log2d + 1)) + (qc & (dil - 1));
+    };
     int voffA, voffB;
     if (contig) {
         const int pp = pbase - 32 + 4 * (lane & 31);
@@ -321,27 +351,33 @@
         }
     };
 
-    bx_f32x16 acc[2][4];
+    Acc acc[2][4];
     __amdgpu_buffer_rsrc_t rA1 = __builtin_amdgcn_make_buffer_rsrc((void*)a.A1, 0, 2 * C * 4 * C * 2 * NT, 0x00020000);
     const int lane16 = lane * 16;
-    auto load_a1 = [&](v8 (&dst)[2][NT], int kb, int j) {
-#pragma unroll
-        for (int m = 0; m < 2; ++m)
+    auto load_a1 = [&](v8 (&dst)[2][NT], int kb, int j, int m0) {
+#pragma unroll
+        for (int f = 0; f < 2; ++f) {
+            const int rt = SPLIT_M ? mt1[m0] * MI + f : mt1[f];
 #pragma unroll
             for (int t = 0; t < NT; ++t)
 #ifdef BX6_ABL_A_HOT
-                dst[m][t] = __builtin_bit_cast(v8, __builtin_amdgcn_raw_buffer_load_b128(rA1, lane16, ((mt1[m] * NKB * 4) * NT + t) * 1024 + 0 * (kb + j), 0));
+                dst[f][t] = __builtin_bit_cast(v8, __builtin_amdgcn_raw_buffer_load_b128(rA1, lane16, ((rt * NKB * 4) * NT + t) * 1024 + 0 * (kb + j), 0));
 #else
-                dst[m][t] = __builtin_bit_cast(v8, __builtin_amdgcn_raw_buffer_load_b128(rA1, lane16, (((mt1[m] * NKB + kb) * 4 + j) * NT + t) * 1024, 0));
-#endif
-    };
+                dst[f][t] = __builtin_bit_cast(v8, __builtin_amdgcn_raw_buffer_load_b128(rA1, lane16, (((rt * NKB + kb) * 4 + j) * NT + t) * 1024, 0));
+#endif
+        }
+    };
+    constexpr int SPC = KBC * 4 * MI;
+    constexpr auto unit_kb = [](int st) constexpr { return st / (4 * MI); };
+    constexpr auto unit_j = [](int st) constexpr { return (st / MI) & 3; };
+    constexpr auto unit_m = [](int st) constexpr { return st % MI; };
 
     stage_dma(0);
     if (NCB > 1) stage_dma(1);
     constexpr int PF = BX6_PF(NT);
     v8 a_ring[4][2][NT];
 #pragma unroll
-    for (int s0 = 0; s0 < PF; ++s0) load_a1(a_ring[s0], chunk_of(0) * (KC / 16) + (s0 >> 2), s0 & 3);
+    for (int s0 = 0; s0 < PF; ++s0) load_a1(a_ring[s0], chunk_of(0) * KBC + unit_kb(s0), unit_j(s0), unit_m(s0));
     constexpr int NAF = PF * NA;
     if (NCB > 1) {
         if (x4) __builtin_amdgcn_s_waitcnt(0x0F70 | ((RPW / 2 + NAF) & 15) | (((RPW / 2 + NAF) >> 4) << 14));
@@ -352,24 +388,34 @@
     __syncthreads();
     stamp(1);
     {
-        const float v0 = ((unsigned)(p - dil) < (unsigned)L) ? 1.f : 0.f;
-        const float v1 = ((unsigned)p < (unsigned)L) ? 1.f : 0.f;
-        const float v2 = ((unsigned)(p + dil) < (unsigned)L) ? 1.f : 0.f;
-        const float v3 = ((unsigned)(p + 2 * dil) < (unsigned)L) ? 1.f : 0.f;
-        const float bi[4] = {v0 - v2, v1 + v2, v2 - v1, v1 - v3};
-        bx_f32x16 zero;
-#pragma unroll
-        for (int r = 0; r < 16; ++r) zero[r] = 0.f;
+        float bi[NI][4];
+#pragma unroll
+        for (int ni = 0; ni < NI; ++ni) {
+            const int pp = col_pos(ni);
+            const float v0 = ((unsigned)(pp - dil) < (unsigned)L) ? 1.f : 0.f;
+            const float v1 = ((unsigned)pp < (unsigned)L) ? 1.f : 0.f;
+            const float v2 = ((unsigned)(pp + dil) < (unsigned)L) ? 1.f : 0.f;
+            const float v3 = ((unsigned)(pp + 2 * dil) < (unsigned)L) ? 1.f : 0.f;
+            bi[ni][0] = v0 - v2; bi[ni][1] = v1 + v2; bi[ni][2] = v2 - v1; bi[ni][3] = v1 - v3;
+        }
 #pragma unroll
         for (int j = 0; j < 4; ++j) {
-            const v8 bf = P::bvals(lhi ? 0.f : bi[j] * P::SX, (lhi || j != 1) ? 0.f : P::SX);
+            v8 bf[NI];
+#pragma unroll
+            for (int ni = 0; ni < NI; ++ni) bf[ni] = P::bvals(fko ? 0.f : bi[ni][j] * P::SX, (fko || j != 1) ? 0.f : P::SX);
 #pragma unroll
             for (int m = 0; m < 2; ++m) {
-                v8 af[NT];
-                P::rank2(av1[m][j] * ws1, j == 1 ? ab1[m] * ws1 : 0.f, lhi == 0, af);
-                acc[m][j] = zero;
-#pragma unroll
-                for (int t = NT - 1; t >= 0; --t) acc[m][j] = P::mfma(af[t], bf, acc[m][j]);
+                acc[m][j].clear();
+#pragma unroll
+                for (int mi = 0; mi < MI; ++mi) {
+                    v8 af[NT];
+                    P::rank2(av1[m][mi][j] * ws1, j == 1 ? ab1[m][mi] * ws1 : 0.f, fko == 0, af);
+#pragma unroll
+                    for (int ni = 0; ni < NI; ++ni)
+#pragma unroll
+                        for (int t = NT - 1; t >= 0; --t)
+                            acc[m][j].sub[mi * NI + ni] = M::mfma(af[t], bf[ni], acc[m][j].sub[mi * NI + ni]);
+                }
             }
         }
     }
@@ -377,14 +423,13 @@
     __builtin_amdgcn_s_waitcnt(0x0F70 | NAF);
     __syncthreads();
 
-    constexpr int SPC = (KC / 16) * 4;
     auto do_step = [&](int cb, auto ST, auto WITH_T) {
         constexpr int st = decltype(ST)::value;
         constexpr bool with_t = decltype(WITH_T)::value;
-        constexpr int it = st >> 2, j = st & 3;
-        constexpr int sn = (st + PF) % SPC, itn = sn >> 2, jn = sn & 3;
+        constexpr int it = unit_kb(st), j = unit_j(st), m0 = unit_m(st);
+        constexpr int sn = (st + PF) % SPC;
         const int cbn = cb + (st + PF) / SPC;
-        const char* tb = Bop + (cb & 1) * T::BOP_BYTES + lhi * (4 * NT * 512) + l31 * 16;
+        const char* tb = Bop + (cb & 1) * T::BOP_BYTES + fko * (4 * NT * 512) + frc * 16;
 #if !defined(BX6_ABL_NO_STAGE) && defined(BX6_STAGE_SPREAD)
         if (cb + 2 < NCB) {
             constexpr int NS = (SPC - PF) < 1 ? 1 : (SPC - PF);
@@ -393,25 +438,32 @@
                 if (i * NS / NPIECE == st) stage_piece(cb + 2, i);
         }
 #endif
-        if (cbn < NCB) load_a1(a_ring[(st + PF) & 3], chunk_of(cbn) * (KC / 16) + itn, jn);
+        if (cbn < NCB) load_a1(a_ring[(st + PF) & 3], chunk_of(cbn) * KBC + unit_kb(sn), unit_j(sn), unit_m(sn));
         __builtin_amdgcn_sched_barrier(0);
-        v8 bq[NT];
-#pragma unroll
-        for (int t = 0; t < NT; ++t) bq[t] = *reinterpret_cast<const v8*>(tb + ((2 * it * 4 + j) * NT + t) * 512);
 #ifndef BX6_ABL_NO_TRANSFORM
         if (with_t) transform(cb + 1);
 #endif
 #pragma unroll
-        for (int t = 0; t < NPR; ++t)
-#pragma unroll
-            for (int m = 0; m < 2; ++m)
-                acc[m][j] = P::mfma(a_ring[st & 3][m][P::ia(t)], bq[P::ib(t)], acc[m][j]);
+        for (int ni = 0; ni < NI; ++ni) {
+            v8 bq[NT];
+#pragma unroll
+            for (int t = 0; t < NT; ++t) bq[t] = *reinterpret_cast<const v8*>(tb + ((it * KO * 4 + j) * NT + t) * 512 + ni * (M::TN * 16));
+#pragma unroll
+            for (int t = 0; t < NPR; ++t)
+#pragma unroll
+                for (int f = 0; f < 2; ++f) {
+                    const int mm = SPLIT_M ? m0 : f;
+                    const int ss = SPLIT_M ? f * NI + ni : ni;
+                    acc[mm][j].sub[ss] = M::mfma(a_ring[st & 3][f][P::ia(t)], bq[P::ib(t)], acc[mm][j].sub[ss]);
+                }
+        }
 #ifndef BX6_ABL_NO_INTERLEAVE
         if (with_t) {
-#pragma unroll
-            for (int i = 0; i < 2 * NPR; ++i) {
+            constexpr int TPM = SPLIT_M ? BX6_T_PER_MFMA_K32 : BX6_T_PER_MFMA;
+#pragma unroll
+            for (int i = 0; i < 2 * NI * NPR; ++i) {
                 __builtin_amdgcn_sched_group_barrier(0x008, 1, 0);
-                __builtin_amdgcn_sched_group_barrier(0x302, BX6_T_PER_MFMA * 6 / NPR, 0);
+                __builtin_amdgcn_sched_group_barrier(0x302, TPM * 6 / NPR, 0);
             }
         }
 #endif
@@ -476,24 +528,32 @@
         for (int m = 1; m < 1 + MS; ++m) load_pre(m, pre[PRELOAD ? m : 0]);
     }
 
+    int pc[NI], gcol0[NI], gcol1[NI];
+#pragma unroll
+    for (int ni = 0; ni < NI; ++ni) {
+        pc[ni] = col_pos(ni);
+        gcol0[ni] = contig ? pc[ni] - pbase : M::TN * ni + frc;
+        gcol1[ni] = contig ? pc[ni] - pbase + dil : 32 + M::TN * ni + frc;
+    }
     const float* melb = (EXTRA && a.melc) ? a.melc + (size_t)(a.mel_bstride ? b : 0) * 2 * C * L : nullptr;
 #pragma unroll
     for (int qd = 0; qd < 4; ++qd) {
         float g0[4], g1[4];
+        const int row4 = Acc::row4(lane, qd);
+        const int ci = Acc::ci(qd);
 #pragma unroll
         for (int e = 0; e < 4; ++e) {
-            const int r = qd * 4 + e;
-            const int ch = wave * 32 + e + 8 * qd + 4 * lhi;
+            const int ch = wave * 32 + row4 + e;
 #pragma unroll
             for (int n = 0; n < 2; ++n) {
-                const int pos = p + n * dil;
+                const int pos = pc[ci] + n * dil;
                 float ht, hs;
                 if (n == 0) {
-                    ht = (acc[0][0][r] + acc[0][1][r]) + acc[0][2][r];
-                    hs = (acc[1][0][r] + acc[1][1][r]) + acc[1][2][r];
+                    ht = (acc[0][0].at(qd, e) + acc[0][1].at(qd, e)) + acc[0][2].at(qd, e);
+                    hs = (acc[1][0].at(qd, e) + acc[1][1].at(qd, e)) + acc[1][2].at(qd, e);
                 } else {
-                    ht = (acc[0][1][r] - acc[0][2][r]) - acc[0][3][r];
-                    hs = (acc[1][1][r] - acc[1][2][r]) - acc[1][3][r];
+                    ht = (acc[0][1].at(qd, e) - acc[0][2].at(qd, e)) - acc[0][3].at(qd, e);
+                    hs = (acc[1][1].at(qd, e) - acc[1][2].at(qd, e)) - acc[1][3].at(qd, e);
                 }
                 if (P::SCALED) { ht *= inv1; hs *= inv1; }
                 if (EXTRA && melb && pos < L) {
@@ -512,70 +572,96 @@
         v4 s0[NT], s1[NT];
         P::split4(g0, s0);
         P::split4(g1, s1);
-        char* dst = gt + ((wave * 4 + qd) * NT * 64) * 16 + lhi * 8;
+        char* dst = gt + ((wave * 4 + (row4 >> 3)) * NT * 64) * 16 + ((row4 >> 2) & 1) * 8;
 #pragma unroll
         for (int t = 0; t < NT; ++t) {
-            *reinterpret_cast<v4*>(dst + (t * 64 + gcol0) * 16) = s0[t];
-            *reinterpret_cast<v4*>(dst + (t * 64 + gcol1) * 16) = s1[t];
+            *reinterpret_cast<v4*>(dst + (t * 64 + gcol0[ci]) * 16) = s0[t];
+            *reinterpret_cast<v4*>(dst + (t * 64 + gcol1[ci]) * 16) = s1[t];
         }
     }
     stamp(3);
 
     __amdgpu_buffer_rsrc_t rA2 = __builtin_amdgcn_make_buffer_rsrc((void*)a.A2, 0, (C + S) * C * 2 * NT, 0x00020000);
-    v8 c_cur[1 + MS][NT], c_nxt[1 + MS][NT];
-    auto load_a2 = [&](v8 (&dst)[1 + MS][NT], int kb) {
+    constexpr int UP2 = SPLIT_M ? 1 + MS : 1;
+    constexpr int AF2 = SPLIT_M ? MI : 1 + MS;
+    v8 c_cur[AF2][NT], c_nxt[AF2][NT];
+    auto load_a2 = [&](v8 (&dst)[AF2][NT], int kb, int mu) {
+#pragma unroll
+        for (int f = 0; f < AF2; ++f) {
+            const int rt = SPLIT_M ? mt2[mu] * MI + f : mt2[f];
+#pragma unroll
+            for (int t = 0; t < NT; ++t)
+                dst[f][t] = __builtin_bit_cast(v8, __builtin_amdgcn_raw_buffer_load_b128(rA2, lane16, ((rt * NKB + kb) * NT + t) * 1024, 0));
+        }
+    };
+    const int rot2 = rot * KBC;
+    auto kblock_of = [&](int kb) { const int k = kb + rot2; return k >= NKB ? k - NKB : k; };
+    load_a2(c_cur, kblock_of(0), 0);
+    Acc acc2[1 + MS][2];
+    {
+        float av2[1 + MS][MI];
 #pragma unroll
         for (int m = 0; m < 1 + MS; ++m)
 #pragma unroll
-            for (int t = 0; t < NT; ++t)
-                dst[m][t] = __builtin_bit_cast(v8, __builtin_amdgcn_raw_buffer_load_b128(rA2, lane16, ((mt2[m] * NKB + kb) * NT + t) * 1024, 0));
-    };
-    const int rot2 = rot * (KC / 16);
-    auto kblock_of = [&](int kb) { const int k = kb + rot2; return k >= NKB ? k - NKB : k; };
-    load_a2(c_cur, kblock_of(0));
-    bx_f32x16 acc2[1 + MS][2];
-    {
-        const v8 bf = P::bvals(lhi ? 0.f : P::SG, 0.f);
-        bx_f32x16 zero;
-#pragma unroll
-        for (int r = 0; r < 16; ++r) zero[r] = 0.f;
+            for (int mi = 0; mi < MI; ++mi) av2[m][mi] = a.bias2[mt2[m] * 32 + mi * M::TM + frc];
+        const v8 bf = P::bvals(fko ? 0.f : P::SG, 0.f);
 #pragma unroll
         for (int m = 0; m < 1 + MS; ++m) {
-            v8 af[NT];
-            P::rank2(av2[m] * ws2, 0.f, lhi == 0, af);
-#pragma unroll
-            for (int n = 0; n < 2; ++n) {
-                acc2[m][n] = zero;
-#pragma unroll
-                for (int t = NT - 1; t >= 0; --t) acc2[m][n] = P::mfma(af[t], bf, acc2[m][n]);
+#pragma unroll
+            for (int n = 0; n < 2; ++n) acc2[m][n].clear();
+#pragma unroll
+            for (int mi = 0; mi < MI; ++mi) {
+                v8 af[NT];
+                P::rank2(av2[m][mi] * ws2, 0.f, fko == 0, af);
+#pragma unroll
+                for (int n = 0; n < 2; ++n)
+#pragma unroll
+                    for (int ni = 0; ni < NI; ++ni)
+#pragma unroll
+                        for (int t = NT - 1; t >= 0; --t)
+                            acc2[m][n].sub[mi * NI + ni] = M::mfma(af[t], bf, acc2[m][n].sub[mi * NI + ni]);
             }
         }
     }
     __syncthreads();
     stamp(4);
-    const char* gb = gt + lhi * (NT * 64 * 16) + l31 * 16;
+    const char* gb = gt + fko * (NT * 64 * 16) + frc * 16;
+    v8 bq2[2][NI][NT];
 #pragma unroll 2
     for (int kb = 0; kb < NKB; ++kb) {
         const int kbn = (kb + 1 < NKB) ? kb + 1 : kb;
-        load_a2(c_nxt, kblock_of(kbn));
-        __builtin_amdgcn_sched_barrier(0);
-        const char* gk = gb + kblock_of(kb) * (2 * NT * 64 * 16);
-        v8 bq[2][NT];
-#pragma unroll
-        for (int n = 0; n < 2; ++n)
-#pragma unroll
-            for (int t = 0; t < NT; ++t) bq[n][t] = *reinterpret_cast<const v8*>(gk + (t * 64 + n * 32) * 16);
-#pragma unroll
-        for (int t = 0; t < NPR; ++t)
-#pragma unroll
-            for (int m = 0; m < 1 + MS; ++m)
+#pragma unroll
+        for (int mu = 0; mu < UP2; ++mu) {
+            if (mu + 1 < UP2) load_a2(c_nxt, kblock_of(kb), mu + 1);
+            else load_a2(c_nxt, kblock_of(kbn), 0);
+            __builtin_amdgcn_sched_barrier(0);
+            if (mu == 0) {
+                const char* gk = gb + kblock_of(kb) * (KO * NT * 64 * 16);
 #pragma unroll
                 for (int n = 0; n < 2; ++n)
-                    acc2[m][n] = P::mfma(c_cur[m][P::ia(t)], bq[n][P::ib(t)], acc2[m][n]);
-#pragma unroll
-        for (int m = 0; m < 1 + MS; ++m)
-#pragma unroll
-            for (int t = 0; t < NT; ++t) c_cur[m][t] = c_nxt[m][t];
+#pragma unroll
+                    for (int ni = 0; ni < NI; ++ni)
+#pragma unroll
+                        for (int t = 0; t < NT; ++t)
+                            bq2[n][ni][t] = *reinterpret_cast<const v8*>(gk + (t * 64 + n * 32 + ni * M::TN) * 16);
+            }
+            if (!(SPLIT_M && mu == 0 && last))
+#pragma unroll
+            for (int t = 0; t < NPR; ++t)
+#pragma unroll
+                for (int f = 0; f < AF2; ++f)
+#pragma unroll
+                    for (int n = 0; n < 2; ++n)
+#pragma unroll
+                        for (int ni = 0; ni < NI; ++ni) {
+                            const int mm = SPLIT_M ? mu : f, ss = SPLIT_M ? f * NI + ni : ni;
+                            acc2[mm][n].sub[ss] = M::mfma(c_cur[f][P::ia(t)], bq2[n][ni][P::ib(t)], acc2[mm][n].sub[ss]);
+                        }
+#pragma unroll
+            for (int f = 0; f < AF2; ++f)
+#pragma unroll
+                for (int t = 0; t < NT; ++t) c_cur[f][t] = c_nxt[f][t];
+        }
     }
     stamp(5);
 
@@ -589,7 +675,10 @@
 #pragma unroll
             for (int n = 0; n < 2; ++n)
 #pragma unroll
-                for (int r = 0; r < 16; ++r) trw[((r & 3) + 8 * (r >> 2) + 4 * lhi) * 64 + n * 32 + l31] = P::SCALED ? acc2[m][n][r] * inv2 : acc2[m][n][r];
+                for (int g = 0; g < 4; ++g)
+#pragma unroll
+                    for (int e = 0; e < 4; ++e)
+                        trw[(Acc::row4(lane, g) + e) * 64 + n * 32 + Acc::col(lane, g)] = P::SCALED ? acc2[m][n].at(g, e) * inv2 : acc2[m][n].at(g, e);
             asm volatile("s_waitcnt lgkmcnt(0)" ::: "memory");
             const int row0 = (m == 0) ? wave * 32 : (wave * MS + (m - 1)) * 32;
 #pragma unroll
@@ -603,33 +692,33 @@
             asm volatile("" ::: "memory");
         }
     } else {
-        int voffn[2];
 #pragma unroll
         for (int n = 0; n < 2; ++n) {
-            const int pos = contig ? pbase + 32 * n + l31 : p + n * dil;
-            voffn[n] = (pos < L) ? (4 * lhi * L + pos) * 4 : 0x7ffffff0;
-        }
-#pragma unroll
-        for (int n = 0; n < 2; ++n) {
-            if (!last) {
-                const int s0 = (wave * 32) * L4;
-#pragma unroll
-                for (int r = 0; r < 16; ++r) {
-                    const int so = s0 + ((r & 3) + 8 * (r >> 2)) * L4;
-                    const float x = __builtin_bit_cast(float, __builtin_amdgcn_raw_buffer_load_b32(rXall, voffn[n], so, 0));
-                    const float v = (x + (P::SCALED ? acc2[0][n][r] * inv2 : acc2[0][n][r])) * rs;
-                    __builtin_amdgcn_raw_buffer_store_b32(__builtin_bit_cast(unsigned, v), rXo, voffn[n], so, 0);
-                }
-            }
-#pragma unroll
-            for (int m = 0; m < MS; ++m) {
-                const int s0 = ((wave * MS + m) * 32) * L4;
-#pragma unroll
-                for (int r = 0; r < 16; ++r) {
-                    const int so = s0 + ((r & 3) + 8 * (r >> 2)) * L4;
-                    const float old = first ? 0.f : __builtin_bit_cast(float, __builtin_amdgcn_raw_buffer_load_b32(rSk, voffn[n], so, 0));
-                    const float v = old + (P::SCALED ? acc2[1 + m][n][r] * inv2 : acc2[1 + m][n][r]);
-                    __builtin_amdgcn_raw_buffer_store_b32(__builtin_bit_cast(unsigned, v), rSk, voffn[n], so, 0);
+#pragma unroll
+            for (int g = 0; g < 4; ++g) {
+                const int ci = Acc::ci(g);
+                const int pos = contig ? pbase + 32 * n + Acc::col(lane, g) : pc[ci] + n * dil;
+                const int voffn = (pos < L) ? (Acc::row4(lane, g) * L + pos) * 4 : 0x7ffffff0;
+                if (!last) {
+                    const int s0 = (wave * 32) * L4;
+#pragma unroll
+                    for (int e = 0; e < 4; ++e) {
+                        const int so = s0 + e * L4;
+                        const float x = __builtin_bit_cast(float, __builtin_amdgcn_raw_buffer_load_b32(rXall, voffn, so, 0));
+                        const float v = (x + (P::SCALED ? acc2[0][n].at(g, e) * inv2 : acc2[0][n].at(g, e))) * rs;
+                        __builtin_amdgcn_raw_buffer_store_b32(__builtin_bit_cast(unsigned, v), rXo, voffn, so, 0);
+                    }
+                }
+#pragma unroll
+                for (int m = 0; m < MS; ++m) {
+                    const int s0 = ((wave * MS + m) * 32) * L4;
+#pragma unroll
+                    for (int e = 0; e < 4; ++e) {
+                        const int so = s0 + e * L4;
+                        const float old = first ? 0.f : __builtin_bit_cast(float, __builtin_amdgcn_raw_buffer_load_b32(rSk, voffn, so, 0));
+                        const float v = old + (P::SCALED ? acc2[1 + m][n].at(g, e) * inv2 : acc2[1 + m][n].at(g, e));
+                        __builtin_amdgcn_raw_buffer_store_b32(__builtin_bit_cast(unsigned, v), rSk, voffn, so, 0);
+                    }
                 }
             }
         }
@@ -641,7 +730,7 @@
     }
 }
 
-template <typename P, int C, int S>
+template <typename P, typename M, int C, int S>
 static int launch_bx6_t(const WnLayerArgs& a, int log2d, hipStream_t s) {
     ProfileScope ps(P::NT == 3 ? "wn_layer_bx6" : "wn_layer_f16x3", s);
     using T = Bx6Tile<C, S, P::NT>;
@@ -652,12 +741,12 @@
     static const bool trace = std::getenv("DWS_BX6_TRACE") != nullptr;
     if (trace && !a.melc && !a.hsave) {
         wino_trace_launch(ntiles, T::WAVES, a, s, [&](const WnLayerArgs& at) {
-            hipLaunchKernelGGL((wn_layer_bx6_kernel<P, C, S, false>), dim3(ntiles), dim3(T::NTH), 0, s, at, log2d);
+            hipLaunchKernelGGL((wn_layer_bx6_kernel<P, M, C, S, false>), dim3(ntiles), dim3(T::NTH), 0, s, at, log2d);
         }, P::NT == 3 ? "bx6" : "f16x3");
         return DWS_OK;
     }
-    if (a.melc || a.hsave) hipLaunchKernelGGL((wn_layer_bx6_kernel<P, C, S, true>), dim3(ntiles), dim3(T::NTH), 0, s, a, log2d);
-    else hipLaunchKernelGGL((wn_layer_bx6_kernel<P, C, S, false>), dim3(ntiles), dim3(T::NTH), 0, s, a, log2d);
+    if (a.melc || a.hsave) hipLaunchKernelGGL((wn_layer_bx6_kernel<P, M, C, S, true>), dim3(ntiles), dim3(T::NTH), 0, s, a, log2d);
+    else hipLaunchKernelGGL((wn_layer_bx6_kernel<P, M, C, S, false>), dim3(ntiles), dim3(T::NTH), 0, s, a, log2d);
     return DWS_OK;
 }
 
@@ -665,16 +754,18 @@
     return (C == 64 && S == 64) || (C == 128 && S == 128) || (C == 128 && S == 256) || (C == 256 && S == 256);
 }
 
+bool wn_layer_bx6_k32_supported(int C, int S, int split) { return C == 256 && S == 256 && split == WN_SPLIT_BF16X6; }
+
 template <typename P>
 static int launch_bx6_p(int C, int S, const WnLayerArgs& a, int log2d, hipStream_t s) {
-    if (C == 64 && S == 64) return launch_bx6_t<P, 64, 64>(a, log2d, s);
-    if (C == 128 && S == 128) return launch_bx6_t<P, 128, 128>(a, log2d, s);
-    if (C == 128 && S == 256) return launch_bx6_t<P, 128, 256>(a, log2d, s);
-    if (C == 256 && S == 256) return launch_bx6_t<P, 256, 256>(a, log2d, s);
+    if (C == 64 && S == 64) return launch_bx6_t<P, Mfma32x32x16, 64, 64>(a, log2d, s);
+    if (C == 128 && S == 128) return launch_bx6_t<P, Mfma32x32x16, 128, 128>(a, log2d, s);
+    if (C == 128 && S == 256) return launch_bx6_t<P, Mfma32x32x16, 128, 256>(a, log2d, s);
+    if (C == 256 && S == 256) return launch_bx6_t<P, Mfma32x32x16, 256, 256>(a, log2d, s);
     return set_error(DWS_ERR_UNSUPPORTED, "wn_layer_bx6: (C=%d,S=%d) not instantiated", C, S);
 }
 
-int launch_wn_layer_bx6(int C, int S, const WnLayerArgs& a, int split, hipStream_t s) {
+int launch_wn_layer_bx6(int C, int S, const WnLayerArgs& a, int split, hipStream_t s, int mfma) {
     int log2d = 0;
     while ((1 << log2d) < a.dilation) ++log2d;
     DWS_CHECK((1 << log2d) == a.dilation, DWS_ERR_UNSUPPORTED, "wn_layer_bx6: dilation %d is not a power of two", a.dilation);
@@ -682,37 +773,42 @@
     DWS_CHECK((int64_t)(C > S ? C : S) * a.L * 4 < ((int64_t)1 << 31), DWS_ERR_UNSUPPORTED,
               "wn_layer_bx6: %d channels x L=%d exceed a 2 GiB tensor per clip", C > S ? C : S, a.L);
     if (split == WN_SPLIT_F16X3) {
+        DWS_CHECK(mfma == WN_MFMA_32X32X16, DWS_ERR_UNSUPPORTED, "wn_layer_f16x3: no 16x16x32 instance");
         DWS_CHECK(a.hsave == nullptr, DWS_ERR_UNSUPPORTED, "wn_layer_f16x3: the training forward runs with precision=f32 or bf16x6");
         DWS_CHECK(a.wscale != nullptr, DWS_ERR_INVALID, "wn_layer_f16x3: no weight scales");
         return launch_bx6_p<SplitF16x2>(C, S, a, log2d, s);
     }
+    if (mfma == WN_MFMA_16X16X32) {
+        DWS_CHECK(wn_layer_bx6_k32_supported(C, S, split), DWS_ERR_UNSUPPORTED, "wn_layer_bx6: no 16x16x32 instance for (C=%d,S=%d)", C, S);
+        return launch_bx6_t<SplitBf16x3, Mfma16x16x32, 256, 256>(a, log2d, s);
+    }
     return launch_bx6_p<SplitBf16x3>(C, S, a, log2d, s);
 }
 
-template <typename P>
+template <typename P, typename M>
 __global__ __launch_bounds__(64) void gemm_bx6_kernel(const float* __restrict__ A, const float* __restrict__ B, float* __restrict__ Cm,
-                                                      int M, int N, int K, float sa, float sb) {
+                                                      int Mr, int N, int K, float sa, float sb) {
     using v8 = typename P::v8;
-    const int lane = threadIdx.x, l31 = lane & 31, lhi = lane >> 5;
+    const int lane = threadIdx.x, frc = M::rc(lane), fko = M::ko(lane);
     const int mt = blockIdx.y, nt = blockIdx.x;
-    bx_f32x16 acc;
-#pragma unroll
-    for (int r = 0; r < 16; ++r) acc[r] = 0.f;
-    for (int kb = 0; kb < K / 16; ++kb) {
+    typename M::acc_t acc;
+#pragma unroll
+    for (int r = 0; r < M::ACCN; ++r) acc[r] = 0.f;
+    for (int kb = 0; kb < K / M::TK; ++kb) {
         v8 af[P::NT], bf[P::NT];
 #pragma unroll
         for (int e = 0; e < 8; ++e) {
-            const int k = kb * 16 + 8 * lhi + e;
-            P::split1(A[(size_t)(mt * 32 + l31) * K + k] * sa, af, e);
-            P::split1(B[(size_t)k * N + nt * 32 + l31] * sb, bf, e);
-        }
-#pragma unroll
-        for (int t = 0; t < P::NP; ++t) acc = P::mfma(af[P::ia(t)], bf[P::ib(t)], acc);
+            const int k = kb * M::TK + 8 * fko + e;
+            P::split1(A[(size_t)(mt * M::TM + frc) * K + k] * sa, af, e);
+            P::split1(B[(size_t)k * N + nt * M::TN + frc] * sb, bf, e);
+        }
+#pragma unroll
+        for (int t = 0; t < P::NP; ++t) acc = M::mfma(af[P::ia(t)], bf[P::ib(t)], acc);
     }
     const float inv = 1.f / (sa * sb);
 #pragma unroll
-    for (int r = 0; r < 16; ++r)
-        Cm[(size_t)(mt * 32 + (r & 3) + 8 * (r >> 2) + 4 * lhi) * N + nt * 32 + l31] = acc[r] * inv;
+    for (int r = 0; r < M::ACCN; ++r)
+        Cm[(size_t)(mt * M::TM + M::arow(lane, r)) * N + nt * M::TN + frc] = acc[r] * inv;
 }
 
 int launch_gemm_bx6(const float* A, const float* B, float* Cm, int M, int N, int K, int split, float sa, float sb, hipStream_t s) {
@@ -722,13 +818,26 @@
         int ea = 0, eb = 0;
         DWS_CHECK(sa > 0.f && sb > 0.f && frexpf(sa, &ea) == 0.5f && frexpf(sb, &eb) == 0.5f, DWS_ERR_INVALID,
                   "gemm_f16x3: the operand scales must be powers of two (%g, %g)", (double)sa, (double)sb);
-        hipLaunchKernelGGL(gemm_bx6_kernel<SplitF16x2>, dim3(N / 32, M / 32), dim3(64), 0, s, A, B, Cm, M, N, K, sa, sb);
+        hipLaunchKernelGGL((gemm_bx6_kernel<SplitF16x2, Mfma32x32x16>), dim3(N / 32, M / 32), dim3(64), 0, s, A, B, Cm, M, N, K, sa, sb);
     } else {
-        hipLaunchKernelGGL(gemm_bx6_kernel<SplitBf16x3>, dim3(N / 32, M / 32), dim3(64), 0, s, A, B, Cm, M, N, K, 1.f, 1.f);
+        hipLaunchKernelGGL((gemm_bx6_kernel<SplitBf16x3, Mfma32x32x16>), dim3(N / 32, M / 32), dim3(64), 0, s, A, B, Cm, M, N, K, 1.f, 1.f);
     }
     return DWS_OK;
 }
 
+int launch_gemm_bx6_k32(const float* A, const float* B, float* Cm, int M, int N, int K, hipStream_t s) {
+    DWS_CHECK(M > 0 && N > 0 && K > 0 && M % 16 == 0 && N % 16 == 0 && K % 32 == 0, DWS_ERR_UNSUPPORTED,
+              "gemm_bf16x6_k32: M=%d N=%d must be multiples of 16, K=%d of 32", M, N, K);
+    hipLaunchKernelGGL((gemm_bx6_kernel<SplitBf16x3, Mfma16x16x32>), dim3(N / 16, M / 16), dim3(64), 0, s, A, B, Cm, M, N, K, 1.f, 1.f);
+    return DWS_OK;
+}
+
+}
+
+extern "C" int dws_gemm_bf16x6_k32(const float* A, const float* B, float* C, int64_t M, int64_t N, int64_t K, void* stream) {
+    DWS_CHECK(A && B && C, DWS_ERR_INVALID, "dws_gemm_bf16x6_k32: null argument");
+    DWS_CHECK(M <= (1 << 20) && N <= (1 << 20) && K <= (1 << 20), DWS_ERR_UNSUPPORTED, "dws_gemm_bf16x6_k32: dimension too large");
+    return dws::launch_gemm_bx6_k32(A, B, C, (int)M, (int)N, (int)K, (hipStream_t)stream);
 }
 
 extern "C" int dws_gemm_bf16x6(const float* A, const float* B, float* C, int64_t M, int64_t N, int64_t K, void* stream) {
diff --git a/diffwave-sashimi_amd/csrc/wavenet_model.hip b/diffwave-sashimi_amd/csrc/wavenet_model.hip
--- a/diffwave-sashimi_amd/csrc/wavenet_model.hip
+++ b/diffwave-sashimi_amd/csrc/wavenet_model.hip
@@ -13,6 +13,7 @@
     bool bf16x3 = false;
     bool bf16x6 = false;
     bool f16x3 = false;
+    int bx6_mfma = -1;
     DevBuf wscale;
     bool wino_opt = true;
     bool wino_fits(int64_t nL) const {
@@ -101,23 +102,37 @@
 
     int set_option(const std::string& key, const std::string& value) override {
         if (key == "precision") {
-            if (value == "f32") { bf16x3 = bf16x6 = f16x3 = false; dirty = true; trained_fwd = false; return DWS_OK; }
+            if (value == "f32") { bf16x3 = bf16x6 = f16x3 = false; bx6_mfma = -1; dirty = true; trained_fwd = false; return DWS_OK; }
             if (value == "bf16x3") {
                 DWS_CHECK(wn_layer_bf16x3_supported(C, S), DWS_ERR_UNSUPPORTED,
                           "precision=bf16x3 is not built for (res_channels=%d, skip_channels=%d)", C, S);
-                bf16x3 = true; bf16x6 = f16x3 = false; dirty = true; trained_fwd = false;
+                bf16x3 = true; bf16x6 = f16x3 = false; bx6_mfma = -1; dirty = true; trained_fwd = false;
                 return DWS_OK;
             }
             if (value == "bf16x6") {
                 DWS_CHECK(mfma_layer && wn_layer_bx6_supported(C, S), DWS_ERR_UNSUPPORTED,
                           "precision=bf16x6 is not built for (res_channels=%d, skip_channels=%d)", C, S);
-                bf16x6 = true; bf16x3 = f16x3 = false; dirty = true; trained_fwd = false;
+                bf16x6 = true; bf16x3 = f16x3 = false; bx6_mfma = -1; dirty = true; trained_fwd = false;
                 return DWS_OK;
             }
             if (value == "f16x3") {
                 DWS_CHECK(mfma_layer && wn_layer_bx6_supported(C, S), DWS_ERR_UNSUPPORTED,
                           "precision=f16x3 is not built for (res_channels=%d, skip_channels=%d)", C, S);
-                f16x3 = true; bf16x3 = bf16x6 = false; dirty = true; trained_fwd = false;
+                f16x3 = true; bf16x3 = bf16x6 = false; bx6_mfma = -1; dirty = true; trained_fwd = false;
+                return DWS_OK;
+            }
+        }
+        if (key == "bx6_mfma") {
+            if (value == "32x32x16") {
+                DWS_CHECK(bf16x6 || f16x3, DWS_ERR_UNSUPPORTED, "bx6_mfma applies to precision=bf16x6 / f16x3");
+                bx6_mfma = WN_MFMA_32X32X16; dirty = true; trained_fwd = false;
+                return DWS_OK;
+            }
+            if (value == "16x16x32") {
+                DWS_CHECK(bf16x6 && wn_layer_bx6_k32_supported(C, S, WN_SPLIT_BF16X6), DWS_ERR_UNSUPPORTED,
+                          "bx6_mfma=16x16x32 is built for precision=bf16x6 at res_channels = skip_channels = 256 (here %d, %d%s)", C, S,
+                          bf16x6 ? "" : ", another precision");
+                bx6_mfma = WN_MFMA_16X16X32; dirty = true; trained_fwd = false;
                 return DWS_OK;
             }
         }
@@ -126,6 +141,10 @@
             if (value == "direct") { wino_opt = false; dirty = true; trained_fwd = false; return DWS_OK; }
         }
         return dws_model::set_option(key, value);
+    }
+
+    bool k32() const {
+        return bf16x6 && (bx6_mfma < 0 ? wn_layer_bx6_k32_supported(C, S, WN_SPLIT_BF16X6) : bx6_mfma == WN_MFMA_16X16X32);
     }
 
     float* Wd(int n) const { return Wd_all.f() + (size_t)n * 2 * C * C * 3; }
@@ -168,8 +187,13 @@
                 }
                 DWS_TRY(A1[n].ensure((size_t)2 * C * 4 * C * tb));
                 DWS_TRY(A2[n].ensure((size_t)(C + S) * C * tb));
-                DWS_TRY(launch_pack_a1_bx6(Wd(n), A1[n].p, C, split, sc, s));
-                DWS_TRY(launch_pack_a_bx6(Wrs[n].f(), A2[n].p, C + S, C, split, f16x3 ? sc + 1 : nullptr, s));
+                if (k32()) {
+                    DWS_TRY(launch_pack_a1_bx6_k32(Wd(n), A1[n].p, C, s));
+                    DWS_TRY(launch_pack_a_bx6_k32(Wrs[n].f(), A2[n].p, C + S, C, s));
+                } else {
+                    DWS_TRY(launch_pack_a1_bx6(Wd(n), A1[n].p, C, split, sc, s));
+                    DWS_TRY(launch_pack_a_bx6(Wrs[n].f(), A2[n].p, C + S, C, split, f16x3 ? sc + 1 : nullptr, s));
+                }
             } else if (mfma_layer) {
                 DWS_TRY(A1[n].ensure((size_t)2 * C * 4 * C * 4));
                 if (wino()) DWS_TRY(launch_wino_dconv(Wd(n), tmp_pack.f(), C, s));
@@ -446,7 +470,7 @@
             a.dilation = 1 << (n % cycle);
             a.first_layer = (n == 0); a.last_layer = (n == NL - 1);
             if (mfma_layer && bf16x3) DWS_TRY(launch_wn_layer_bf16x3(C, S, a, s));
-            else if (bf16x6) DWS_TRY(launch_wn_layer_bx6(C, S, a, WN_SPLIT_BF16X6, s));
+            else if (bf16x6) DWS_TRY(launch_wn_layer_bx6(C, S, a, WN_SPLIT_BF16X6, s, k32() ? WN_MFMA_16X16X32 : WN_MFMA_32X32X16));
             else if (f16x3) { a.wscale = wscale.f() + 2 * n; DWS_TRY(launch_wn_layer_bx6(C, S, a, WN_SPLIT_F16X3, s)); }
             else if (wino()) DWS_TRY(launch_wn_layer_wino(C, S, a, s));
             else if (mfma_layer) DWS_TRY(launch_wn_layer_mfma(C, S, a, s));
diff --git a/include/dws.h b/include/dws.h
--- a/include/dws.h
+++ b/include/dws.h
@@ -126,6 +126,8 @@
 
 int dws_gemm_bf16x6(const float* A, const float* B, float* C, int64_t M, int64_t N, int64_t K, void* stream);
 
+int dws_gemm_bf16x6_k32(const float* A, const float* B, float* C, int64_t M, int64_t N, int64_t K, void* stream);
+
 int dws_gemm_f16x3(const float* A, const float* B, float* C, int64_t M, int64_t N, int64_t K, float scale_a, float scale_b,
                    void* stream);
 
```

Result: no change. 32790 audio samples/s, median of 6 (+0.3%).
